# GestaltCogTeam/STEP

Measured on AMD Instinct MI355X. Metric: training windows/sec on PEMS04, horizon-12 MAE parity, 1/2/4/8 MI355X, higher is better.
Workload: dtype f16 (TSFormer Q/K/weights) + bf16 (P, V, GraphWaveNet / graph-learner GEMMs) operands, f32 accumulate

## Files before the change

include/step_hip.h:

```cpp
#ifndef STEP_HIP_H
#define STEP_HIP_H

#include <stdint.h>

#ifdef __cplusplus
extern "C" {
#endif

const char* step_last_error(void);
int step_abi_version(void);

typedef struct StepGemm {
    int M, N, K, batch;
    const void* A; long sam, sak, sab; int a_bf16;
    const void* B; long sbk, sbn, sbb; int b_bf16;
    float* C; long ldc, scn, scb;
    float alpha;
    int accumulate;
    const float* bias; int relu;
    int splitk;
    int a_kblk; long a_kstride;
    int b_kblk; long b_kstride;
    int b_nblk; long b_nstride;
    int c_nblk; long c_nstride;
// ... 13 lines not shown
#define STEP_ENC_WORKGROUPS(n) (((n) & 0xffff) << 8)
int step_tsformer_encode(const float* series, int S, int L, const void* wpack, long wpack_bytes,
                         int depth, int flags, uint16_t* hidden_bf16, float* hidden_f32, float* last_f32,
                         float* sqnorm_part, float dropout_p, const uint64_t* drop_pool, long pool_words, uint64_t seed,
                         unsigned int* fallback_count, void* stream);
int step_dropout_pool_fill(uint64_t* pool, long words, float dropout_p, uint64_t seed, void* stream);
long step_tsformer_dropout_words(int L, int depth);

int step_pack_long_history(const float* x, int B, int L, int N, int C, int ch, float* out, void* stream);
int step_gather_windows(const float* data, int T, int N, int C, int ch, const long* t0, int B, int L, int H,
                        float* long_series, float* hist, float* fut, void* stream);

long step_knn_workspace_bytes(int B, int N, int F);
int step_knn_graph(const uint16_t* hidden, const float* sqnorm_part, int B, int N, int F, int k_total,
                   float* sim, float* adj, void* work, long work_bytes, void* stream);
int step_topk_mask(const float* sim, int B, int N, int k_total, float* adj, void* work, long work_bytes,
                   void* stream);

typedef struct StepDglParams {
    float *conv1_w, *conv1_b;
    float *conv2_w, *conv2_b;
    float *fc_w, *fc_b;
    float *bn1_w, *bn1_b, *bn1_rm, *bn1_rv;
    float *bn2_w, *bn2_b, *bn2_rm, *bn2_rv;
    float *bn3_w, *bn3_b, *bn3_rm, *bn3_rv;
    float *fc_out_w, *fc_out_b;
    float *fc_cat_w, *fc_cat_b;
    int gemm_bf16;
} StepDglParams;

long step_dgl_global_saved_floats(int N, int T);
long step_dgl_global_work_floats(int N, int T, int backward);
int step_dgl_global_forward(const float* series_nt, int N, int T, const StepDglParams* p, int training,
                            float momentum, float* saved, float* work, float* g, void* stream);
int step_dgl_global_backward(const float* series_nt, int N, int T, const StepDglParams* p, const float* saved,
                             const float* dg, float* work, const StepDglParams* grads, void* stream);
#define STEP_DGL_FRESH_FC_GRAD 16
int step_dgl_global_backward_phase(const float* series_nt, int N, int T, const StepDglParams* p, const float* saved,
                             const float* dg, float* work, const StepDglParams* grads, int phase, void* stream);

typedef struct StepDglShard { int own1; double count1, count2; } StepDglShard;
int step_dgl_global_forward_shard(const float* series_slice, int N, int Ts, const StepDglParams* p, int training, float momentum,
                                  float* saved, float* work, double* sums, float* g, const StepDglShard* shard, int phase,
                                  void* stream);
int step_dgl_global_backward_shard(const float* series_slice, int N, int Ts, const StepDglParams* p, const float* saved,
                                   const float* dg, float* work, const StepDglParams* grads, const StepDglShard* shard, int phase,
                                   void* stream);
long step_dgl_global_offset(int N, int T, int item);

long step_dgl_edges_saved_floats(int B, int N);
long step_dgl_edges_work_floats(int N);
long step_dgl_edges_theta_offset(int N);
int step_dgl_edges_forward(const float* g, int N, int B, const StepDglParams* p, const float* u, uint64_t seed,
                           float temperature, float* saved, float* theta_out, float* adj_out, void* stream);
int step_dgl_edges_backward(const float* g, int N, int B, const StepDglParams* p, const float* saved,
                            const float* dtheta, const float* dadj, float temperature, float* work,
                            const StepDglParams* grads, float* dg, void* aux_stream, void* stream);

typedef struct StepGwnetParams {
    float *nodevec1, *nodevec2;
    float *start_w, *start_b;
    float *filter_w[8], *filter_b[8];
    float *gate_w[8], *gate_b[8];
    float *skip_w[8], *skip_b[8];
    float *bn_w[8], *bn_b[8], *bn_rm[8], *bn_rv[8];
    float *gconv_w[8], *gconv_b[8];
    float *fc_his0_w, *fc_his0_b, *fc_his2_w, *fc_his2_b;
    float *end1_w, *end1_b, *end2_w, *end2_b;
    int gemm_bf16;
} StepGwnetParams;

long step_gwnet_saved_floats(int B, int N, int dropout);
long step_gwnet_work_floats(int B, int N, int backward);
long step_gwnet_saved_offset(int B, int N, int dropout, int item, int layer);
int step_gwnet_forward(const float* hist, int B, int N, int Cin, const float* hidden_last, const float* adj,
                       const StepGwnetParams* p, int training, float dropout_p, uint64_t seed, float momentum,
                       float* saved, float* work, float* pred, void* stream);
int step_gwnet_forward_phase(const float* hist, int B, int N, int Cin, const float* hidden_last, const float* adj,
                             const StepGwnetParams* p, int training, float dropout_p, uint64_t seed, float momentum,
                             float* saved, float* work, float* pred, int phase, void* stream);
int step_gwnet_backward(const float* hist, int B, int N, int Cin, const float* hidden_last, const StepGwnetParams* p,
                        const float* saved, float* work, const float* dpred, const StepGwnetParams* grads,
                        float* dadj, int dropout, void* aux_stream, void* leaf_stream, void* stream);

int step_pt_dropout(const float* x, float* y, long n, float p, uint64_t seed, uint32_t site, void* stream);
int step_pt_ffn_hidden_fwd(const float* x, const float* w1, const float* b1, long R, float p, uint64_t seed, uint32_t site,
                           uint16_t* hidden, void* stream);
int step_pt_ffn_hidden_bwd(const float* dy, const float* w2, const uint16_t* hidden, long R, float p, uint16_t* dhidden, void* stream);
int step_pt_colsum_bf16(const uint16_t* x, long rows, int cols, float* out, void* stream);
long step_pt_rows_linear_pack_bytes(int nkc, int nog);
int step_pt_rows_linear_pack(const float* w, long swo, long swi, int nkc, int nog, const float* bias, void* pack, void* stream);
int step_pt_rows_linear(const void* x, int x_bf16, long R, const void* pack, int nkc, int nog, void* y, int y_bf16, int accumulate, void* stream);
int step_pt_layer_pack(const float* wi, const float* bi, const float* wo, const float* bo, const float* w1, const float* b1, const float* w2,
                       const float* b2, void* ffn, void* qkv, void* o, void* da, void* dx, void* stream);
long step_pt_proj_wgrad_ws_floats(long R);
int step_pt_proj_wgrad(const float* x, const uint16_t* dqkv, const float* dov, const uint16_t* a, long R, float* ws, float* dwi, float* dbi, float* dwo,
                       void* stream);
int step_pt_ffn_fused_fwd_ln(const float* h1, long R, const void* pack, float p, const uint64_t* pool, long pool_words, uint64_t seed, uint32_t site_hidden,
                             uint32_t site_out, const float* gamma, const float* beta, float* pre, float* y, float* stats, void* stream);
int step_pt_rows_linear_ln(const uint16_t* x, long R, const void* pack, const float* res, float p, uint64_t seed, uint32_t site, const float* gamma,
                           const float* beta, float* pre, float* y, float* stats, void* stream);
int step_pt_embed_unmasked_fwd(const float* series, const int* um, const float* w, const float* b, const float* pos, long S, int L, int Pu, float p,
                               uint64_t seed, uint32_t site, float* x, void* stream);
int step_pt_embed_unmasked_bwd(const float* dx, const float* series, const int* um, long S, int L, int Pu, float p, uint64_t seed, uint32_t site,
                               float* dpos, float* dw, float* db, void* stream);
int step_pt_dec_input_bwd_sums(const float* dout, long S, int P, int Pu, float p, uint64_t seed, uint32_t site, const int* midx, float* dz, float* dpos,
                               float* dmask, void* stream);
long step_pt_ffn_pack_bytes(void);
long step_pt_ffn_wgrad_workgroups(long R);
long step_pt_ffn_wgrad_ws_floats(long R);
int step_pt_ffn_pack(const float* w1, const float* b1, const float* w2, const float* b2, void* pack, void* stream);
int step_pt_ffn_fused_fwd(const float* h1, long R, const void* pack, float p, const uint64_t* pool, long pool_words, uint64_t seed, uint32_t site,
                          float* f2, void* stream);
int step_pt_ffn_fused_bwd_data(const float* df2, const float* h1, long R, const void* pack, float p, const uint64_t* pool, long pool_words,
                               uint64_t seed, uint32_t site, float* dh1, void* stream);
int step_pt_ffn_fused_bwd_weights(const float* df2, const float* h1, long R, const void* pack, const float* b1, float p, const uint64_t* pool,
                                  long pool_words, uint64_t seed, uint32_t site, float* ws, float* dw1, float* db1, float* dw2, void* stream);
int step_pt_dropout_relu_mask(float* d, const float* relu_of, long n, float p, uint64_t seed, uint32_t site, void* stream);
int step_pt_add_dropout(const float* a, const float* b, float* out, long n, float p, uint64_t seed, uint32_t site, void* stream);
int step_pt_add_rows(float* x, long S, int P, const float* vec, const int* idx, void* stream);
int step_pt_sum_over_seq(const float* dx, long S, int ldp, int p_off, int p_cnt, const int* idx, float* dvec, void* stream);
int step_pt_token_gather(const float* src, long S, int P, const int* idx, int T, float scale, float* dst, void* stream);
int step_pt_token_scatter(const float* ddst, long S, int P, const int* idx, int T, float scale, float* dsrc, void* stream);
int step_pt_dec_input(const float* z, const float* mask_token, const float* pos, const int* midx, long S, int P, int Pu,
                      float p, uint64_t seed, uint32_t site, float* out, void* stream);
int step_pt_dec_input_bwd(const float* dout, long S, int P, int Pu, float p, uint64_t seed, uint32_t site, float* dz,
                          float* dm, void* stream);
int step_pt_layernorm_fwd(const float* x, long R, const float* g, const float* b, float* y, float* stats, void* stream);
int step_pt_layernorm_bwd(const float* dy, const float* x, long R, const float* g, const float* stats, float* dx, float* dgamma,
                          float* dbeta, void* stream);
int step_pt_add_layernorm_fwd(const float* a, const float* b, long R, float p, uint64_t seed, uint32_t site, const float* g,
                              const float* beta, float* pre, float* y, float* stats, void* stream);
int step_pt_layernorm_bwd_dropout(const float* dy, const float* x, long R, const float* g, const float* stats, float* dx,
                                  float* dx_dropped, float p, uint64_t seed, uint32_t site, float* dgamma, float* dbeta,
                                  float* out_colsum, void* stream);
int step_pt_attention_fwd(const float* qkv, long S, int T, float p, uint64_t seed, uint32_t site, float* out, float* stats,
                          void* stream);
int step_pt_attention_bwd(const float* qkv, const float* out, const float* dout, const float* stats, long S, int T, float p,
                          uint64_t seed, uint32_t site, float* dqkv, void* stream);
int step_pt_attention_fwd_bf16(const uint16_t* qkv, long S, int T, float p, uint64_t seed, uint32_t site, uint16_t* out, float* stats,
                               uint32_t* keepbits, const uint64_t* pool, long pool_words, void* stream);
int step_pt_attention_bwd_bf16(const uint16_t* qkv, const uint16_t* out, const uint16_t* dout, const float* stats, long S, int T, float p,
                               uint64_t seed, uint32_t site, uint16_t* dqkv, const uint32_t* keepbits, void* stream);
int step_pt_linear_bf16out(const float* x, const float* w, long swk, long swn, const float* bias, long R, int N, int K, uint16_t* out,
                           void* stream);
int step_pt_relu_mask(float* d, const float* y, long n, void* stream);
int step_colsum(const float* x, long rows, int cols, long ld, float* out, void* stream);

long step_adam_work_floats(void);
int step_adam_clip(float* params, const float* grads, float* exp_avg, float* exp_avg_sq, long n, float lr, float beta1,
                   float beta2, float eps, float weight_decay, int step, float max_norm, float* work, float* out_norm,
                   void* stream);
int step_adam_clip_sharded(float* params, const float* grads, float* exp_avg, float* exp_avg_sq, long n, float lr, float beta1,
                           float beta2, float eps, float weight_decay, int step, float max_norm, const float* extra_sumsq,
                           float* work, float* out_norm, void* stream);
int step_loss_fwd_bwd(const float* pred, const float* real, long n_pred, const float* theta, const float* prior, long n_adj,
                      float null_val, float coef, double* work, float* loss, float* dpred, float* dtheta, void* stream);
int step_loss_scaled_fwd_bwd(const float* pred, const float* real, long n_pred, long real_stride, float scale, float shift,
                             const float* theta, const float* prior, long n_adj, float null_val, float coef, double* work, float* loss,
                             float* dpred, float* dtheta, void* stream);
int step_masked_metrics(const float* pred, long pred_stride, const float* real, long real_stride, long n, float null_val, double* work,
                        float* out, void* stream);
int step_scale2(const float* a, long na, const float* b, long nb, const float* g, float* out_a, float* out_b, void* stream);

typedef struct StepDynState {
    uint64_t seed_xor;
    int32_t adam_step;
    float lr;
    float gsl_coef;
    float reserved;
} StepDynState;
int step_dyn_advance(StepDynState* dyn, void* stream);
int step_dropout_pool_fill_dyn(uint64_t* pool, long words, float dropout_p, uint64_t seed, const StepDynState* dyn, void* stream);
int step_dgl_edges_forward_dyn(const float* g, int N, int B, const StepDglParams* p, const float* u, uint64_t seed,
                               float temperature, float* saved, float* theta_out, float* adj_out, const StepDynState* dyn, void* stream);
int step_gwnet_forward_phase_dyn(const float* hist, int B, int N, int Cin, const float* hidden_last, const float* adj,
                                 const StepGwnetParams* p, int training, float dropout_p, uint64_t seed, float momentum,
                                 float* saved, float* work, float* pred, int phase, const StepDynState* dyn, void* stream);
int step_adam_clip_dyn(float* params, const float* grads, float* exp_avg, float* exp_avg_sq, long n, float beta1, float beta2, float eps,
                       float weight_decay, float max_norm, const float* extra_sumsq, float* work, float* out_norm,
                       const StepDynState* dyn, void* stream);
int step_loss_scaled_fwd_bwd_dyn(const float* pred, const float* real, long n_pred, long real_stride, float scale, float shift,
                                 const float* theta, const float* prior, long n_adj, float null_val, double* work, float* loss,
                                 float* dpred, float* dtheta, const StepDynState* dyn, void* stream);

#define STEP_COMM_ID_BYTES 128
#define STEP_COMM_F32 0
#define STEP_COMM_F64 1
#define STEP_COMM_U8 2
int step_comm_available(void);
int step_comm_version(void);
int step_comm_unique_id(void* id128);
int step_comm_init_rank(const void* id128, int nranks, int rank, void** comm_out);
int step_comm_destroy(void* comm);
int step_comm_set_side_stream(void* comm, void* stream);
int step_comm_allreduce(void* comm, void* buf, long n, int dtype, int average, void* stream);
int step_comm_broadcast(void* comm, void* buf, long n, int dtype, int root, void* stream);
int step_grad_allreduce(void* comm, float* flat_grad, long n, void* stream);
int step_grad_allreduce_begin(void* comm, float* flat_grad, long n, void* stream);
int step_grad_allreduce_join(void* comm, void* stream);

int step_frozen_cache_store(const float* last, const float* adj, int B, int N, const long* slot, long capacity,
                            float* cache_last, uint32_t* cache_bits, void* stream);
int step_frozen_cache_load(const float* cache_last, const uint32_t* cache_bits, long capacity, const long* slot, int B, int N,
                           float* last, float* adj, void* stream);

long step_eval_metrics_acc_doubles(int H);
int step_eval_metrics_accumulate(const float* pred, long p_sb, long p_sh, long p_sn, const float* real, long r_sb, long r_sh, long r_sn,
                                 int B, int H, int N, float scale, float shift, float null_val, double* acc, void* stream);
int step_eval_metrics_finish(const double* acc, int H, double* out, void* stream);

long step_train_tail_work_doubles(void);
int step_train_tail(const float* pred, long p_sb, long p_sh, long p_sn, const float* real, long r_sb, long r_sh, long r_sn, int B, int H,
                    int N, int k, float scale, float shift, float null_val, const float* theta, const float* prior, long n_adj, float coef,
                    double* work, float* loss, float* metrics, float* dpred, float* dtheta, void* stream);

int step_selftest_mfma(int32_t* out, void* stream);
int step_streams_concurrent(void* stream_a, void* stream_b, int* concurrent);

#ifdef __cplusplus
}
#endif
#endif
```

step_amd/_lib.py:

```python
import ctypes
import os

import torch

_HERE = os.path.dirname(os.path.abspath(__file__))
LIB_PATH = os.environ.get("STEP_HIP_LIB") or os.path.join(_HERE, "libstep_hip.so")

_vp, _i, _l, _f, _u64 = ctypes.c_void_p, ctypes.c_int, ctypes.c_long, ctypes.c_float, ctypes.c_uint64


class StepGemm(ctypes.Structure):
    _fields_ = [("M", _i), ("N", _i), ("K", _i), ("batch", _i),
                ("A", _vp), ("sam", _l), ("sak", _l), ("sab", _l), ("a_bf16", _i),
                ("B", _vp), ("sbk", _l), ("sbn", _l), ("sbb", _l), ("b_bf16", _i),
                ("C", _vp), ("ldc", _l), ("scn", _l), ("scb", _l),
                ("alpha", _f), ("accumulate", _i), ("bias", _vp), ("relu", _i), ("splitk", _i),
                ("a_kblk", _i), ("a_kstride", _l), ("b_kblk", _i), ("b_kstride", _l),
                ("b_nblk", _i), ("b_nstride", _l), ("c_nblk", _i), ("c_nstride", _l),
                ("a_kscale", _vp), ("a_kshift", _vp), ("a_kperiod", _i),
                ("batch0", _i), ("sab1", _l), ("sbb1", _l), ("scb1", _l), ("compute_bf16", _i), ("a_rowsum", _vp), ("c_nscale", _vp), ("c_nshift", _vp), ("c_mvec", _vp),
                ("c_nperiod", _i), ("splitk_ws", _vp), ("splitk_ws_floats", _l)]


class StepDglParams(ctypes.Structure):
    NAMES = ["conv1_w", "conv1_b", "conv2_w", "conv2_b", "fc_w", "fc_b",
             "bn1_w", "bn1_b", "bn1_rm", "bn1_rv", "bn2_w", "bn2_b", "bn2_rm", "bn2_rv",
             "bn3_w", "bn3_b", "bn3_rm", "bn3_rv", "fc_out_w", "fc_out_b", "fc_cat_w", "fc_cat_b"]
    _fields_ = [(n, _vp) for n in NAMES] + [("gemm_bf16", _i)]


class StepGwnetParams(ctypes.Structure):
    _fields_ = [("nodevec1", _vp), ("nodevec2", _vp), ("start_w", _vp), ("start_b", _vp),
                ("filter_w", _vp * 8), ("filter_b", _vp * 8), ("gate_w", _vp * 8), ("gate_b", _vp * 8),
                ("skip_w", _vp * 8), ("skip_b", _vp * 8),
                ("bn_w", _vp * 8), ("bn_b", _vp * 8), ("bn_rm", _vp * 8), ("bn_rv", _vp * 8),
                ("gconv_w", _vp * 8), ("gconv_b", _vp * 8),
                ("fc_his0_w", _vp), ("fc_his0_b", _vp), ("fc_his2_w", _vp), ("fc_his2_b", _vp),
                ("end1_w", _vp), ("end1_b", _vp), ("end2_w", _vp), ("end2_b", _vp), ("gemm_bf16", _i)]


_PD = ctypes.POINTER(StepDglParams)


class StepDynState(ctypes.Structure):
    _fields_ = [("seed_xor", ctypes.c_uint64), ("adam_step", ctypes.c_int32), ("lr", _f), ("gsl_coef", _f), ("reserved", _f)]


class StepDglShard(ctypes.Structure):
    _fields_ = [("own1", ctypes.c_int), ("count1", ctypes.c_double), ("count2", ctypes.c_double)]


_PS = ctypes.POINTER(StepDglShard)
_PG = ctypes.POINTER(StepGwnetParams)

_SIGS = {
    "step_last_error": (ctypes.c_char_p, []),
    "step_abi_version": (_i, []),
    "step_gemm": (_i, [ctypes.POINTER(StepGemm), _vp]),
    "step_tsformer_encode": (_i, [_vp, _i, _i, _vp, _l, _i, _i, _vp, _vp, _vp, _vp, _f, _vp, _l, _u64, _vp, _vp]),
    "step_dropout_pool_fill": (_i, [_vp, _l, _f, _u64, _vp]),
    "step_tsformer_dropout_words": (_l, [_i, _i]),
    "step_gather_windows": (_i, [_vp, _i, _i, _i, _i, _vp, _i, _i, _i, _vp, _vp, _vp, _vp]),
    "step_pack_long_history": (_i, [_vp, _i, _i, _i, _i, _i, _vp, _vp]),
    "step_knn_workspace_bytes": (_l, [_i, _i, _i]),
    "step_knn_graph": (_i, [_vp, _vp, _i, _i, _i, _i, _vp, _vp, _vp, _l, _vp]),
    "step_topk_mask": (_i, [_vp, _i, _i, _i, _vp, _vp, _l, _vp]),
    "step_selftest_mfma": (_i, [_vp, _vp]),
    "step_streams_concurrent": (_i, [_vp, _vp, ctypes.POINTER(_i)]),
    "step_dgl_global_saved_floats": (_l, [_i, _i]),
    "step_dgl_global_work_floats": (_l, [_i, _i, _i]),
    "step_dgl_global_forward": (_i, [_vp, _i, _i, _PD, _i, _f, _vp, _vp, _vp, _vp]),
    "step_dgl_global_backward": (_i, [_vp, _i, _i, _PD, _vp, _vp, _vp, _PD, _vp]),
    "step_dgl_global_backward_phase": (_i, [_vp, _i, _i, _PD, _vp, _vp, _vp, _PD, _i, _vp]),
    "step_dgl_global_forward_shard": (_i, [_vp, _i, _i, _PD, _i, _f, _vp, _vp, _vp, _vp, _PS, _i, _vp]),
    "step_dgl_global_backward_shard": (_i, [_vp, _i, _i, _PD, _vp, _vp, _vp, _PD, _PS, _i, _vp]),
    "step_dgl_global_offset": (_l, [_i, _i, _i]),
    "step_dgl_edges_saved_floats": (_l, [_i, _i]),
    "step_dgl_edges_work_floats": (_l, [_i]),
    "step_dgl_edges_theta_offset": (_l, [_i]),
    "step_dgl_edges_forward": (_i, [_vp, _i, _i, _PD, _vp, _u64, _f, _vp, _vp, _vp, _vp]),
    "step_dgl_edges_backward": (_i, [_vp, _i, _i, _PD, _vp, _vp, _vp, _f, _vp, _PD, _vp, _vp, _vp]),
    "step_gwnet_saved_floats": (_l, [_i, _i, _i]),
    "step_gwnet_work_floats": (_l, [_i, _i, _i]),
    "step_gwnet_saved_offset": (_l, [_i, _i, _i, _i, _i]),
    "step_gwnet_forward": (_i, [_vp, _i, _i, _i, _vp, _vp, _PG, _i, _f, _u64, _f, _vp, _vp, _vp, _vp]),
    "step_gwnet_forward_phase": (_i, [_vp, _i, _i, _i, _vp, _vp, _PG, _i, _f, _u64, _f, _vp, _vp, _vp, _i, _vp]),
    "step_gwnet_backward": (_i, [_vp, _i, _i, _i, _vp, _PG, _vp, _vp, _vp, _PG, _vp, _i, _vp, _vp, _vp]),
    "step_pt_dropout": (_i, [_vp, _vp, _l, _f, _u64, ctypes.c_uint32, _vp]),
    "step_pt_ffn_hidden_fwd": (_i, [_vp, _vp, _vp, _l, _f, _u64, ctypes.c_uint32, _vp, _vp]),
    "step_pt_ffn_hidden_bwd": (_i, [_vp, _vp, _vp, _l, _f, _vp, _vp]),
    "step_pt_colsum_bf16": (_i, [_vp, _l, _i, _vp, _vp]),
    "step_pt_rows_linear_pack_bytes": (_l, [_i, _i]),
    "step_pt_rows_linear_pack": (_i, [_vp, _l, _l, _i, _i, _vp, _vp, _vp]),
    "step_pt_rows_linear": (_i, [_vp, _i, _l, _vp, _i, _i, _vp, _i, _i, _vp]),
    "step_pt_layer_pack": (_i, [_vp] * 14),
    "step_pt_proj_wgrad_ws_floats": (_l, [_l]),
    "step_pt_proj_wgrad": (_i, [_vp, _vp, _vp, _vp, _l, _vp, _vp, _vp, _vp, _vp]),
    "step_pt_ffn_fused_fwd_ln": (_i, [_vp, _l, _vp, _f, _vp, _l, _u64, ctypes.c_uint32, ctypes.c_uint32, _vp, _vp, _vp, _vp, _vp, _vp]),
    "step_pt_rows_linear_ln": (_i, [_vp, _l, _vp, _vp, _f, _u64, ctypes.c_uint32, _vp, _vp, _vp, _vp, _vp, _vp]),
    "step_pt_embed_unmasked_fwd": (_i, [_vp, _vp, _vp, _vp, _vp, _l, _i, _i, _f, _u64, ctypes.c_uint32, _vp, _vp]),
    "step_pt_embed_unmasked_bwd": (_i, [_vp, _vp, _vp, _l, _i, _i, _f, _u64, ctypes.c_uint32, _vp, _vp, _vp, _vp]),
    "step_pt_dec_input_bwd_sums": (_i, [_vp, _l, _i, _i, _f, _u64, ctypes.c_uint32, _vp, _vp, _vp, _vp, _vp]),
    "step_pt_ffn_pack_bytes": (_l, []),
    "step_pt_ffn_wgrad_workgroups": (_l, [_l]),
    "step_pt_ffn_wgrad_ws_floats": (_l, [_l]),
    "step_pt_ffn_pack": (_i, [_vp, _vp, _vp, _vp, _vp, _vp]),
    "step_pt_ffn_fused_fwd": (_i, [_vp, _l, _vp, _f, _vp, _l, _u64, ctypes.c_uint32, _vp, _vp]),
    "step_pt_ffn_fused_bwd_data": (_i, [_vp, _vp, _l, _vp, _f, _vp, _l, _u64, ctypes.c_uint32, _vp, _vp]),
    "step_pt_ffn_fused_bwd_weights": (_i, [_vp, _vp, _l, _vp, _vp, _f, _vp, _l, _u64, ctypes.c_uint32, _vp, _vp, _vp, _vp, _vp]),
    "step_pt_add_layernorm_fwd": (_i, [_vp, _vp, _l, _f, _u64, ctypes.c_uint32, _vp, _vp, _vp, _vp, _vp, _vp]),
    "step_pt_layernorm_bwd_dropout": (_i, [_vp, _vp, _l, _vp, _vp, _vp, _vp, _f, _u64, ctypes.c_uint32, _vp, _vp, _vp, _vp]),
    "step_pt_dropout_relu_mask": (_i, [_vp, _vp, _l, _f, _u64, ctypes.c_uint32, _vp]),
    "step_pt_add_dropout": (_i, [_vp, _vp, _vp, _l, _f, _u64, ctypes.c_uint32, _vp]),
    "step_pt_add_rows": (_i, [_vp, _l, _i, _vp, _vp, _vp]),
    "step_pt_sum_over_seq": (_i, [_vp, _l, _i, _i, _i, _vp, _vp, _vp]),
    "step_pt_token_gather": (_i, [_vp, _l, _i, _vp, _i, _f, _vp, _vp]),
    "step_pt_token_scatter": (_i, [_vp, _l, _i, _vp, _i, _f, _vp, _vp]),
    "step_pt_dec_input": (_i, [_vp, _vp, _vp, _vp, _l, _i, _i, _f, _u64, ctypes.c_uint32, _vp, _vp]),
    "step_pt_dec_input_bwd": (_i, [_vp, _l, _i, _i, _f, _u64, ctypes.c_uint32, _vp, _vp, _vp]),
    "step_pt_layernorm_fwd": (_i, [_vp, _l, _vp, _vp, _vp, _vp, _vp]),
    "step_pt_layernorm_bwd": (_i, [_vp, _vp, _l, _vp, _vp, _vp, _vp, _vp, _vp]),
    "step_pt_attention_fwd": (_i, [_vp, _l, _i, _f, _u64, ctypes.c_uint32, _vp, _vp, _vp]),
    "step_pt_attention_bwd": (_i, [_vp, _vp, _vp, _vp, _l, _i, _f, _u64, ctypes.c_uint32, _vp, _vp]),
    "step_pt_attention_fwd_bf16": (_i, [_vp, _l, _i, _f, _u64, ctypes.c_uint32, _vp, _vp, _vp, _vp, _l, _vp]),
    "step_pt_attention_bwd_bf16": (_i, [_vp, _vp, _vp, _vp, _l, _i, _f, _u64, ctypes.c_uint32, _vp, _vp, _vp]),
    "step_pt_linear_bf16out": (_i, [_vp, _vp, _l, _l, _vp, _l, _i, _i, _vp, _vp]),
    "step_pt_relu_mask": (_i, [_vp, _vp, _l, _vp]),
    "step_colsum": (_i, [_vp, _l, _i, _l, _vp, _vp]),
    "step_loss_fwd_bwd": (_i, [_vp, _vp, _l, _vp, _vp, _l, _f, _f, _vp, _vp, _vp, _vp, _vp]),
    "step_loss_scaled_fwd_bwd": (_i, [_vp, _vp, _l, _l, _f, _f, _vp, _vp, _l, _f, _f, _vp, _vp, _vp, _vp, _vp]),
    "step_scale2": (_i, [_vp, _l, _vp, _l, _vp, _vp, _vp, _vp]),
    "step_masked_metrics": (_i, [_vp, _l, _vp, _l, _l, _f, _vp, _vp, _vp]),
    "step_adam_work_floats": (_l, []),
    "step_adam_clip": (_i, [_vp, _vp, _vp, _vp, _l, _f, _f, _f, _f, _f, _i, _f, _vp, _vp, _vp]),
    "step_adam_clip_sharded": (_i, [_vp, _vp, _vp, _vp, _l, _f, _f, _f, _f, _f, _i, _f, _vp, _vp, _vp, _vp]),
    "step_comm_available": (_i, []),
    "step_comm_version": (_i, []),
    "step_comm_unique_id": (_i, [_vp]),
    "step_comm_init_rank": (_i, [_vp, _i, _i, ctypes.POINTER(_vp)]),
    "step_comm_destroy": (_i, [_vp]),
    "step_comm_set_side_stream": (_i, [_vp, _vp]),
    "step_comm_allreduce": (_i, [_vp, _vp, _l, _i, _i, _vp]),
    "step_comm_broadcast": (_i, [_vp, _vp, _l, _i, _i, _vp]),
    "step_grad_allreduce": (_i, [_vp, _vp, _l, _vp]),
    "step_grad_allreduce_begin": (_i, [_vp, _vp, _l, _vp]),
    "step_grad_allreduce_join": (_i, [_vp, _vp]),
    "step_dyn_advance": (_i, [_vp, _vp]),
    "step_dropout_pool_fill_dyn": (_i, [_vp, _l, _f, _u64, _vp, _vp]),
    "step_dgl_edges_forward_dyn": (_i, [_vp, _i, _i, _PD, _vp, _u64, _f, _vp, _vp, _vp, _vp, _vp]),
    "step_gwnet_forward_phase_dyn": (_i, [_vp, _i, _i, _i, _vp, _vp, _PG, _i, _f, _u64, _f, _vp, _vp, _vp, _i, _vp, _vp]),
    "step_adam_clip_dyn": (_i, [_vp, _vp, _vp, _vp, _l, _f, _f, _f, _f, _f, _vp, _vp, _vp, _vp, _vp]),
    "step_loss_scaled_fwd_bwd_dyn": (_i, [_vp, _vp, _l, _l, _f, _f, _vp, _vp, _l, _f, _vp, _vp, _vp, _vp, _vp, _vp]),
    "step_frozen_cache_store": (_i, [_vp, _vp, _i, _i, _vp, _l, _vp, _vp, _vp]),
    "step_frozen_cache_load": (_i, [_vp, _vp, _l, _vp, _i, _i, _vp, _vp, _vp]),
    "step_eval_metrics_acc_doubles": (_l, [_i]),
    "step_eval_metrics_accumulate": (_i, [_vp, _l, _l, _l, _vp, _l, _l, _l, _i, _i, _i, _f, _f, _f, _vp, _vp]),
    "step_eval_metrics_finish": (_i, [_vp, _i, _vp, _vp]),
    "step_train_tail_work_doubles": (_l, []),
    "step_train_tail": (_i, [_vp, _l, _l, _l, _vp, _l, _l, _l, _i, _i, _i, _i, _f, _f, _f, _vp, _vp, _l, _f, _vp, _vp, _vp, _vp, _vp, _vp]),
}

_lib = None


ABI_VERSION = 10
ENC_F16, ENC_ALWAYS_RESHIFT, ENC_RANGE_FLAG = 1, 2, 4
COMM_F32, COMM_F64, COMM_U8, COMM_ID_BYTES = 0, 1, 2, 128


def lib():
    global _lib
    if _lib is None:
        if not os.path.exists(LIB_PATH):
            raise RuntimeError(
                f"libstep_hip.so not found at {LIB_PATH}: build it with `python -m step_amd.build` "
                "(step_amd has no fallback path)")
        _lib = ctypes.CDLL(LIB_PATH)
        for name, (res, args) in _SIGS.items():
            fn = getattr(_lib, name)
            fn.restype = res
            fn.argtypes = args
        if _lib.step_abi_version() != ABI_VERSION:
            v = _lib.step_abi_version()
            _lib = None
            raise RuntimeError(f"libstep_hip.so has ABI version {v}, this package needs {ABI_VERSION}: rebuild with `python -m step_amd.build`")
    return _lib


def exported_symbols():
    return sorted(_SIGS)


def check(rc, what=""):
    if rc != 0:
        msg = lib().step_last_error().decode(errors="replace")
        raise RuntimeError(f"libstep_hip {what} failed (rc={rc}): {msg}")


def ptr(t):
    if t is None:
        return None
    assert t.is_cuda and t.is_contiguous(), "libstep_hip takes contiguous device tensors"
    return ctypes.c_void_p(t.data_ptr())


def stream():
    return ctypes.c_void_p(torch.cuda.current_stream().cuda_stream)


def call(name, *args):
    check(getattr(lib(), name)(*args), name)


# ... 31 lines not shown
```

step_amd/csrc/dgl.hip:

```cpp
#include "common.h"
#include "step_internal.h"

namespace {

constexpr int KW = 10;
constexpr int EMB = 100;

template <int CI, int CO, int TPT>
__global__ __launch_bounds__(256) void conv_relu_fwd_kernel(const float* __restrict__ in, const float* __restrict__ w,
                                                            const float* __restrict__ b, const float* __restrict__ in_sc,
                                                            const float* __restrict__ in_sh, float* __restrict__ out,
                                                            float* __restrict__ partial, int Tin, int stat_limit) {
    __shared__ __attribute__((aligned(16))) float ws[CI * KW * CO];
    __shared__ float red[4][2 * CO];
    const int tid = threadIdx.x, n = blockIdx.y;
    const int Tout = Tin - (KW - 1);
    for (int e = tid; e < CI * KW * CO; e += 256) {
        int co = e % CO, k = (e / CO) % KW, ci = e / (CO * KW);
        ws[e] = w[(co * CI + ci) * KW + k];
    }
    __syncthreads();
    const int t0 = (blockIdx.x * 256 + tid) * TPT;
    float acc[CO][TPT];
#pragma unroll
    for (int co = 0; co < CO; ++co)
#pragma unroll
        for (int j = 0; j < TPT; ++j) acc[co][j] = b[co];
    if (t0 < Tout) {
#pragma unroll 1
        for (int ci = 0; ci < CI; ++ci) {
            const float* src = in + ((long)n * CI + ci) * Tin + t0;
            const float sc = in_sc ? in_sc[ci] : 1.f, sh = in_sh ? in_sh[ci] : 0.f;
            float x[TPT + KW - 1];
#pragma unroll
            for (int q = 0; q < TPT + KW - 1; ++q) x[q] = (t0 + q < Tin) ? src[q] * sc + sh : 0.f;
#pragma unroll
            for (int k = 0; k < KW; ++k) {
                const float* wk = ws + (ci * KW + k) * CO;
#pragma unroll
                for (int co = 0; co < CO; ++co) {
                    const float wv = wk[co];
#pragma unroll
                    for (int j = 0; j < TPT; ++j) acc[co][j] += wv * x[k + j];
                }
            }
        }
    }
    float s1[CO], s2[CO];
#pragma unroll
    for (int co = 0; co < CO; ++co) {
        s1[co] = 0.f; s2[co] = 0.f;
        float* dst = out + ((long)n * CO + co) * Tout + t0;
#pragma unroll
        for (int j = 0; j < TPT; ++j) {
            if (t0 + j < Tout) {
                float v = fmaxf(acc[co][j], 0.f);
                dst[j] = v;
                if (t0 + j < stat_limit) { s1[co] += v; s2[co] += v * v; }
            }
        }
    }
    const int lane = tid & 63, wave = tid >> 6;
#pragma unroll
    for (int co = 0; co < CO; ++co) {
        float a = wave_sum(s1[co]), q = wave_sum(s2[co]);
        if (lane == 0) { red[wave][co] = a; red[wave][CO + co] = q; }
    }
    __syncthreads();
    if (tid < 2 * CO)
        partial[((long)blockIdx.y * gridDim.x + blockIdx.x) * (2 * CO) + tid] = red[0][tid] + red[1][tid] + red[2][tid] + red[3][tid];
}

__global__ __launch_bounds__(256) void bn_finalize_kernel(const float* __restrict__ partial, int nblk, int C, double count,
                                                          const float* __restrict__ gamma, const float* __restrict__ beta,
                                                          float* __restrict__ rmean, float* __restrict__ rvar, int training,
                                                          float momentum, float* __restrict__ stat) {
    __shared__ double r1[256], r2[256];
    const int c = blockIdx.x, tid = threadIdx.x;
    double mean, var;
    if (training) {
        double a = 0.0, q = 0.0;
        for (int i = tid; i < nblk; i += 256) { a += partial[(long)i * 2 * C + c]; q += partial[(long)i * 2 * C + C + c]; }
        r1[tid] = a; r2[tid] = q;
        __syncthreads();
        for (int s = 128; s > 0; s >>= 1) {
            if (tid < s) { r1[tid] += r1[tid + s]; r2[tid] += r2[tid + s]; }
            __syncthreads();
        }
        mean = r1[0] / count;
        var = fmax(r2[0] / count - mean * mean, 0.0);
        if (tid == 0) {
            rmean[c] = (1.f - momentum) * rmean[c] + momentum * (float)mean;
            rvar[c] = (1.f - momentum) * rvar[c] + momentum * (float)(var * count / fmax(count - 1.0, 1.0));
        }
    } else {
        mean = rmean[c];
        var = rvar[c];
    }
    if (tid == 0) {
        float rstd = (float)(1.0 / sqrt(var + 1e-5));
        float sc = gamma[c] * rstd;
        stat[c] = sc;
        stat[C + c] = beta[c] - (float)mean * sc;
        stat[2 * C + c] = (float)mean;
        stat[3 * C + c] = rstd;
    }
}

__global__ __launch_bounds__(256) void bn_sums_kernel(const float* __restrict__ partial, int nblk, int C, double* __restrict__ sums) {
    __shared__ double r1[256], r2[256];
    const int c = blockIdx.x, tid = threadIdx.x;
    double a = 0.0, q = 0.0;
    for (int i = tid; i < nblk; i += 256) { a += partial[(long)i * 2 * C + c]; q += partial[(long)i * 2 * C + C + c]; }
    r1[tid] = a; r2[tid] = q;
    __syncthreads();
    for (int s = 128; s > 0; s >>= 1) {
        if (tid < s) { r1[tid] += r1[tid + s]; r2[tid] += r2[tid + s]; }
        __syncthreads();
    }
    if (tid == 0) { sums[c] = r1[0]; sums[C + c] = r2[0]; }
}
__global__ __launch_bounds__(256) void bn_sums_sliced_kernel(const float* __restrict__ partial, int nblk, int C, double* __restrict__ sums) {
    __shared__ double r1[256], r2[256];
    const int c = blockIdx.x, tid = threadIdx.x;
    const int per = (nblk + gridDim.y - 1) / gridDim.y, beg = blockIdx.y * per, end = min(nblk, beg + per);
    double a = 0.0, q = 0.0;
    for (int i = beg + tid; i < end; i += 256) { a += partial[(long)i * 2 * C + c]; q += partial[(long)i * 2 * C + C + c]; }
    r1[tid] = a; r2[tid] = q;
    __syncthreads();
    for (int s = 128; s > 0; s >>= 1) {
        if (tid < s) { r1[tid] += r1[tid + s]; r2[tid] += r2[tid + s]; }
        __syncthreads();
    }
    if (tid == 0) { unsafeAtomicAdd(sums + c, r1[0]); unsafeAtomicAdd(sums + C + c, r2[0]); }
}
__global__ void bn_finalize_sums_kernel(const double* __restrict__ sums, int C, double count, const float* __restrict__ gamma,
                                        const float* __restrict__ beta, float* __restrict__ rmean, float* __restrict__ rvar,
                                        int training, float momentum, float* __restrict__ stat) {
    const int c = threadIdx.x;
    if (c >= C) return;
    double mean, var;
    if (training) {
        mean = sums[c] / count;
        var = fmax(sums[C + c] / count - mean * mean, 0.0);
        rmean[c] = (1.f - momentum) * rmean[c] + momentum * (float)mean;
        rvar[c] = (1.f - momentum) * rvar[c] + momentum * (float)(var * count / fmax(count - 1.0, 1.0));
    } else {
        mean = rmean[c]; var = rvar[c];
    }
    const float rstd = (float)(1.0 / sqrt(var + 1e-5));
    const float sc = gamma[c] * rstd;
    stat[c] = sc; stat[C + c] = beta[c] - (float)mean * sc; stat[2 * C + c] = (float)mean; stat[3 * C + c] = rstd;
}

__global__ __launch_bounds__(256) void fc_post_bn3_kernel(float* __restrict__ gpre, const float* __restrict__ bias, int N,
                                                          const float* __restrict__ gamma, const float* __restrict__ beta,
                                                          float* __restrict__ rmean, float* __restrict__ rvar, int training,
                                                          float momentum, float* __restrict__ stat, float* __restrict__ g) {
    __shared__ double r1[256], r2[256];
    const int j = blockIdx.x, tid = threadIdx.x;
    const float bj = bias[j];
    double a = 0.0, q = 0.0;
    for (int n = tid; n < N; n += 256) {
        float v = gpre[(long)n * EMB + j] + bj;
        gpre[(long)n * EMB + j] = v;
        v = fmaxf(v, 0.f);
        a += v; q += (double)v * v;
    }
    r1[tid] = a; r2[tid] = q;
    __syncthreads();
    for (int s = 128; s > 0; s >>= 1) {
        if (tid < s) { r1[tid] += r1[tid + s]; r2[tid] += r2[tid + s]; }
        __syncthreads();
    }
    double mean, var;
    if (training) {
        mean = r1[0] / N;
        var = fmax(r2[0] / N - mean * mean, 0.0);
        if (tid == 0) {
            rmean[j] = (1.f - momentum) * rmean[j] + momentum * (float)mean;
            rvar[j] = (1.f - momentum) * rvar[j] + momentum * (float)(var * N / fmax((double)N - 1.0, 1.0));
        }
    } else {
        mean = rmean[j]; var = rvar[j];
    }
    const float rstd = (float)(1.0 / sqrt(var + 1e-5));
    if (tid == 0) { stat[2 * EMB + j] = (float)mean; stat[3 * EMB + j] = rstd; }
    const float sc = gamma[j] * rstd, sh = beta[j] - (float)mean * sc;
    for (int n = tid; n < N; n += 256) g[(long)n * EMB + j] = fmaxf(gpre[(long)n * EMB + j], 0.f) * sc + sh;
}

__global__ __launch_bounds__(256) void bn3_relu_bwd_kernel(const float* __restrict__ dg, const float* __restrict__ gpre, int N,
                                                           const float* __restrict__ gamma, const float* __restrict__ stat,
                                                           float* __restrict__ dgamma, float* __restrict__ dbeta,
                                                           float* __restrict__ dbias, float* __restrict__ dgpre,
                                                           float* __restrict__ dgpreT, float* __restrict__ colsum) {
    __shared__ double r1[256], r2[256];
    const int j = blockIdx.x, tid = threadIdx.x;
    const float mean = stat[2 * EMB + j], rstd = stat[3 * EMB + j];
    double a = 0.0, q = 0.0;
    for (int n = tid; n < N; n += 256) {
        float d = dg[(long)n * EMB + j];
        float xh = (fmaxf(gpre[(long)n * EMB + j], 0.f) - mean) * rstd;
        a += d; q += (double)d * xh;
    }
    r1[tid] = a; r2[tid] = q;
    __syncthreads();
    for (int s = 128; s > 0; s >>= 1) {
        if (tid < s) { r1[tid] += r1[tid + s]; r2[tid] += r2[tid + s]; }
        __syncthreads();
    }
    const float m1 = (float)(r1[0] / N), m2 = (float)(r2[0] / N);
    const float k = gamma[j] * rstd;
    __syncthreads();
    double sb = 0.0;
    for (int n = tid; n < N; n += 256) {
        float pre = gpre[(long)n * EMB + j];
        float xh = (fmaxf(pre, 0.f) - mean) * rstd;
        float dh = k * (dg[(long)n * EMB + j] - m1 - xh * m2);
        float v = pre > 0.f ? dh : 0.f;
        dgpre[(long)n * EMB + j] = v;
        dgpreT[(long)j * N + n] = v;
        sb += v;
    }
    if (tid == 0) { dgamma[j] += (float)r2[0]; dbeta[j] += (float)r1[0]; }
    __syncthreads();
    r1[tid] = sb;
    __syncthreads();
    for (int s = 128; s > 0; s >>= 1) {
        if (tid < s) r1[tid] += r1[tid + s];
        __syncthreads();
    }
    if (tid == 0) { dbias[j] += (float)r1[0]; colsum[j] = (float)r1[0]; }
}

template <int C>
__global__ __launch_bounds__(256) void bn_bwd_reduce_kernel(const float* __restrict__ dy, const float* __restrict__ x,
                                                            const float* __restrict__ stat, int Tlen, float* __restrict__ partial) {
    __shared__ float red[4][2];
    const int n = blockIdx.z, c = blockIdx.y, tid = threadIdx.x;
    const float mean = stat[2 * C + c], rstd = stat[3 * C + c];
    const long base = ((long)n * C + c) * Tlen;
    float a = 0.f, q = 0.f;
    for (int t = blockIdx.x * 1024 + tid; t < min(Tlen, (int)(blockIdx.x + 1) * 1024); t += 256) {
        float d = dy[base + t];
        a += d; q += d * ((x[base + t] - mean) * rstd);
    }
    a = wave_sum(a); q = wave_sum(q);
    if ((tid & 63) == 0) { red[tid >> 6][0] = a; red[tid >> 6][1] = q; }
    __syncthreads();
    if (tid < 2) {
        long blk = (long)n * gridDim.x + blockIdx.x;
        partial[(blk * C + c) * 2 + tid] = red[0][tid] + red[1][tid] + red[2][tid] + red[3][tid];
    }
}
__global__ __launch_bounds__(256) void bn_bwd_finalize_kernel(const float* __restrict__ partial, int nblk, int C, double count,
                                                              const float* __restrict__ gamma, const float* __restrict__ stat,
                                                              float* __restrict__ dgamma, float* __restrict__ dbeta,
                                                              float* __restrict__ coef) {
    __shared__ double r1[256], r2[256];
    const int c = blockIdx.x, tid = threadIdx.x;
    double a = 0.0, q = 0.0;
    for (int i = tid; i < nblk; i += 256) { a += partial[((long)i * C + c) * 2]; q += partial[((long)i * C + c) * 2 + 1]; }
    r1[tid] = a; r2[tid] = q;
    __syncthreads();
    for (int s = 128; s > 0; s >>= 1) {
        if (tid < s) { r1[tid] += r1[tid + s]; r2[tid] += r2[tid + s]; }
        __syncthreads();
    }
    if (tid == 0) {
        dgamma[c] += (float)r2[0];
        dbeta[c] += (float)r1[0];
        coef[c] = (float)(r1[0] / count);
        coef[C + c] = (float)(r2[0] / count);
        coef[2 * C + c] = gamma[c] * stat[3 * C + c];
    }
}
template <int C>
__global__ __launch_bounds__(256) void bn_bwd_apply_kernel(float* __restrict__ dy, const float* __restrict__ x,
                                                           const float* __restrict__ stat, const float* __restrict__ coef, int Tlen) {
    const int n = blockIdx.z, c = blockIdx.y;
// ... 358 lines not shown
__global__ void gpre_init_kernel(float* __restrict__ gpre, const float* __restrict__ shiftdot, long n) {
    const long i = (long)blockIdx.x * 256 + threadIdx.x;
    if (i < n) gpre[i] = shiftdot[i % EMB];
}
__global__ __launch_bounds__(256) void fc_unpermute_kernel(const float* __restrict__ graw, const float* __restrict__ fc_w,
                                                           const float* __restrict__ st2, const float* __restrict__ colsum,
                                                           float* __restrict__ dfc_w, float* __restrict__ dots_o, int T2, int overwrite) {
    __shared__ float red[4][32];
    const int o = blockIdx.y, t = blockIdx.x * 256 + threadIdx.x, tid = threadIdx.x;
    const float cso = colsum[o];
    float d[32];
#pragma unroll
    for (int i = 0; i < 32; ++i) d[i] = 0.f;
    if (t < T2) {
        const float4* src = (const float4*)(graw + ((long)o * T2 + t) * 16);
        const float4 g0 = src[0], g1 = src[1], g2 = src[2], g3 = src[3];
        const float g[16] = {g0.x, g0.y, g0.z, g0.w, g1.x, g1.y, g1.z, g1.w, g2.x, g2.y, g2.z, g2.w, g3.x, g3.y, g3.z, g3.w};
        float w[16], old[16];
#pragma unroll
        for (int c = 0; c < 16; ++c) { const long idx = ((long)o * 16 + c) * T2 + t; w[c] = fc_w[idx]; old[c] = overwrite ? 0.f : dfc_w[idx]; }
#pragma unroll
        for (int c = 0; c < 16; ++c) {
            dfc_w[((long)o * 16 + c) * T2 + t] = old[c] + st2[c] * g[c] + st2[16 + c] * cso;
            d[2 * c] = w[c] * g[c]; d[2 * c + 1] = w[c] * cso;
        }
    }
#pragma unroll
    for (int i = 0; i < 32; ++i) {
        const float v = wave_sum(d[i]);
        if ((tid & 63) == 0) red[tid >> 6][i] = v;
    }
    __syncthreads();
    if (tid < 32) atomicAdd(&dots_o[o * 32 + tid], red[0][tid] + red[1][tid] + red[2][tid] + red[3][tid]);
}
__global__ void dots_reduce_kernel(const float* __restrict__ dots_o, float* __restrict__ dots) {
    const int i = threadIdx.x;
    if (i >= 32) return;
    double a = 0.0;
    for (int o = 0; o < EMB; ++o) a += dots_o[o * 32 + i];
    dots[i] = (float)a;
}

static bool dgl_channels_last(const StepDglParams* p) {
    const char* e = getenv("STEP_DGL_F32_STORAGE");
    return p->gemm_bf16 && !(e && e[0] == '1');
}

static bool dgl_legacy_bn_backward() {
    const char* e = getenv("STEP_DGL_LEGACY_BN");
    return e && e[0] == '1';
}

extern "C" long step_dgl_global_saved_floats(int N, int T) {
    long T1 = T - 9, T2 = T - 18;
    return (long)N * 8 * T1 + (long)N * 16 * T2 + (long)N * EMB + 4 * 8 + 4 * 16 + 4 * EMB + (long)EMB * 16 * T2 + 128;
}
static long fc_splitk_ws_floats(int N, int T2) {
    const int splits = step_gemm_auto_splitk(N, EMB, 16 * T2, 1);
    return splits > 1 ? (long)splits * N * EMB + 4 : 0;
}
extern "C" long step_dgl_global_work_floats(int N, int T, int backward) {
    long T1 = T - 9, T2 = T - 18;
    long nb1 = (long)N * cdiv(T1, 1024), nb2 = (long)N * cdiv(T2, 1024);
    long part = (nb1 > nb2 ? nb1 : nb2) * 32 + 64;
    if (!backward) return part + dgl_conv2_pack_floats() + 64 + fc_splitk_ws_floats(N, (int)T2);
    return part + (long)N * 16 * T2 + (long)N * 8 * T1 + (long)EMB * 16 * T2 + 2L * N * EMB + DGL_SMALL + dgl_conv2_wgrad_scratch_floats(N, (int)T1);
}

static float* saved_wp(float* saved, int N, int T) {
    long T1 = T - 9, T2 = T - 18;
    return saved + (long)N * 8 * T1 + (long)N * 16 * T2 + (long)N * EMB + 4 * 8 + 4 * 16 + 4 * EMB;
}
static void carve_saved(float* saved, int N, int T, float** a1, float** a2, float** gpre, float** st1, float** st2, float** st3) {
    long T1 = T - 9, T2 = T - 18;
    *a1 = saved; saved += (long)N * 8 * T1;
    *a2 = saved; saved += (long)N * 16 * T2;
    *gpre = saved; saved += (long)N * EMB;
    *st1 = saved; saved += 4 * 8;
    *st2 = saved; saved += 4 * 16;
    *st3 = saved;
}

static int dgl_bn_stats(const float* partial, int nblk, int C, double count, const float* gamma, const float* beta, float* rm, float* rv,
                        int training, float momentum, float* stat, double* sums, hipStream_t st) {
    if (nblk < 8192) {
        bn_finalize_kernel<<<C, 256, 0, st>>>(partial, nblk, C, count, gamma, beta, rm, rv, training, momentum, stat);
    } else {
        if (hipMemsetAsync(sums, 0, 2 * C * sizeof(double), st) != hipSuccess) { step_set_error("memset failed"); return STEP_ERR_HIP; }
        bn_sums_sliced_kernel<<<dim3(C, 32), 256, 0, st>>>(partial, nblk, C, sums);
        bn_finalize_sums_kernel<<<1, 64, 0, st>>>(sums, C, count, gamma, beta, rm, rv, training, momentum, stat);
    }
    STEP_LAUNCH_CHECK("bn_stats");
    return STEP_OK;
}

static int dgl_global_forward_impl(const float* series_nt, int N, int T, const StepDglParams* p, int training, float momentum,
                                   float* saved, float* work, double* sums, float* g, const StepDglShard* shard, int phase,
                                   hipStream_t st) {
    const int T1 = T - 9, T2 = T - 18;
    float *a1, *a2, *gpre, *st1, *st2, *st3;
    carve_saved(saved, N, T, &a1, &a2, &gpre, &st1, &st2, &st3);
    float* partial = work;
    const bool all = phase == 0;
    const double count1 = shard ? shard->count1 : (double)N * T1, count2 = shard ? shard->count2 : (double)N * T2;
    const bool cl = dgl_channels_last(p);
    const long part_floats = ((long)N * cdiv(T1, 1024) > (long)N * cdiv(T2, 1024) ? (long)N * cdiv(T1, 1024) : (long)N * cdiv(T2, 1024)) * 32 + 64;
    double* own_sums = (double*)(work + part_floats + dgl_conv2_pack_floats());
    float* wp = saved_wp(saved, N, T);
    float* shiftdot = wp + (long)EMB * 16 * T2;
    if (all || phase == 1) {
        int nblk;
        if (cl) {
            STEP_TRY(dgl_conv1_fwd_cl(series_nt, p->conv1_w, p->conv1_b, a1, partial, N, T, shard ? shard->own1 : T1, &nblk, st));
        } else {
            dim3 grid(cdiv(T1, 256 * 4), N);
            conv_relu_fwd_kernel<1, 8, 4><<<grid, 256, 0, st>>>(series_nt, p->conv1_w, p->conv1_b, nullptr, nullptr, a1, partial, T,
                                                                shard ? shard->own1 : T1);
            STEP_LAUNCH_CHECK("conv1");
            nblk = grid.x * grid.y;
        }
        if (shard) bn_sums_kernel<<<8, 256, 0, st>>>(partial, nblk, 8, sums);
        else STEP_TRY(dgl_bn_stats(partial, nblk, 8, count1, p->bn1_w, p->bn1_b, p->bn1_rm, p->bn1_rv, training, momentum, st1, own_sums, st));
        STEP_LAUNCH_CHECK("bn1");
    }
    if (all || phase == 2) {
        if (shard) bn_finalize_sums_kernel<<<1, 64, 0, st>>>(sums, 8, count1, p->bn1_w, p->bn1_b, p->bn1_rm, p->bn1_rv, training, momentum, st1);
        int nblk;
        if (cl) {
            STEP_TRY(dgl_conv2_fwd_cl(a1, p->conv2_w, p->conv2_b, st1, st1 + 8, a2, partial, N, T1, &nblk,
                                      work + part_floats, st));
        } else if (p->gemm_bf16) {
            STEP_TRY(dgl_conv2_fwd_mfma(a1, p->conv2_w, p->conv2_b, st1, st1 + 8, a2, partial, N, T1, &nblk, st));
        } else {
            dim3 grid(cdiv(T2, 256 * 4), N);
            conv_relu_fwd_kernel<8, 16, 4><<<grid, 256, 0, st>>>(a1, p->conv2_w, p->conv2_b, st1, st1 + 8, a2, partial, T1, T2);
            STEP_LAUNCH_CHECK("conv2");
            nblk = grid.x * grid.y;
        }
        if (shard) bn_sums_kernel<<<16, 256, 0, st>>>(partial, nblk, 16, sums + 16);
        else STEP_TRY(dgl_bn_stats(partial, nblk, 16, count2, p->bn2_w, p->bn2_b, p->bn2_rm, p->bn2_rv, training, momentum, st2, own_sums, st));
        STEP_LAUNCH_CHECK("bn2");
    }
    if (all || phase == 3) {
        if (shard) bn_finalize_sums_kernel<<<1, 64, 0, st>>>(sums + 16, 16, count2, p->bn2_w, p->bn2_b, p->bn2_rm, p->bn2_rv, training, momentum, st2);
        const long K = 16L * T2;
        StepGemm gm = gemm_desc(N, EMB, (int)K, a2, K, 1, p->fc_w, 1, K, gpre, EMB);
        if (cl) {
            if (hipMemsetAsync(shiftdot, 0, 128 * sizeof(float), st) != hipSuccess) { step_set_error("memset failed"); return STEP_ERR_HIP; }
            fc_prep_kernel<<<dim3(cdiv(T2, 256), EMB), 256, 0, st>>>(p->fc_w, st2, (uint4*)wp, shiftdot, T2);
            gpre_init_kernel<<<cdiv((long)N * EMB, 256), 256, 0, st>>>(gpre, shiftdot, (long)N * EMB);
            STEP_LAUNCH_CHECK("fc_prep");
            gm.a_bf16 = 1;
            gm.B = wp; gm.b_bf16 = 1;
        } else {
            if (hipMemsetAsync(gpre, 0, (size_t)N * EMB * sizeof(float), st) != hipSuccess) { step_set_error("memset failed"); return STEP_ERR_HIP; }
            gm.a_kscale = st2; gm.a_kshift = st2 + 16; gm.a_kperiod = T2;
        }
        gm.accumulate = 2;
        gm.splitk = -1;
        gm.compute_bf16 = p->gemm_bf16;
        if (fc_splitk_ws_floats(N, T2) > 0) {
            float* ws = work + part_floats + dgl_conv2_pack_floats() + 64;
            gm.splitk_ws = (float*)(((uintptr_t)ws + 15) & ~(uintptr_t)15);
            gm.splitk_ws_floats = fc_splitk_ws_floats(N, T2) - 4;
        }
        STEP_TRY(step_gemm_launch(gm, st));
    }
    if (all || phase == 4) {
        fc_post_bn3_kernel<<<EMB, 256, 0, st>>>(gpre, p->fc_b, N, p->bn3_w, p->bn3_b, p->bn3_rm, p->bn3_rv, training, momentum, st3, g);
        STEP_LAUNCH_CHECK("fc_post_bn3");
    }
    return STEP_OK;
}

extern "C" int step_dgl_global_forward(const float* series_nt, int N, int T, const StepDglParams* p, int training,
                                       float momentum, float* saved, float* work, float* g, void* stream) {
    STEP_REQUIRE(series_nt && p && saved && work && g && N > 0 && T > 18, "dgl_global_forward: bad arguments");
    return dgl_global_forward_impl(series_nt, N, T, p, training, momentum, saved, work, nullptr, g, nullptr, 0, (hipStream_t)stream);
}

extern "C" int step_dgl_global_forward_shard(const float* series_slice, int N, int Ts, const StepDglParams* p, int training,
                                             float momentum, float* saved, float* work, double* sums, float* g,
                                             const StepDglShard* shard, int phase, void* stream) {
    STEP_REQUIRE(series_slice && p && saved && work && sums && g && shard && N > 0 && Ts > 18 && phase >= 1 && phase <= 4,
                 "dgl_global_forward_shard: bad arguments");
    STEP_REQUIRE(shard->own1 > 0 && shard->own1 <= Ts - 9 && shard->count1 > 0 && shard->count2 > 0, "dgl_global_forward_shard: bad shard");
    return dgl_global_forward_impl(series_slice, N, Ts, p, training, momentum, saved, work, sums, g, shard, phase, (hipStream_t)stream);
}

extern "C" long step_dgl_global_offset(int N, int T, int item) {
    const long T1 = T - 9, T2 = T - 18;
    if (item == 0) return 0;
    if (item == 1) return (long)N * 8 * T1;
    if (item == 2) return (long)N * 8 * T1 + (long)N * 16 * T2;
    const long nb1 = (long)N * cdiv(T1, 1024), nb2 = (long)N * cdiv(T2, 1024);
    const long coef = (nb1 > nb2 ? nb1 : nb2) * 32 + 64 + (long)N * 16 * T2 + (long)N * 8 * T1 + (long)EMB * 16 * T2 + 2L * N * EMB;
    if (item == 10) return coef + 256;
    if (item == 11) return coef + 320;
    return -1;
}

static int dgl_global_backward_impl(const float* series_nt, int N, int T, const StepDglParams* p, const float* saved, const float* dg,
                                    float* work, const StepDglParams* grads, const StepDglShard* shard, int phase, void* stream);

extern "C" int step_dgl_global_backward(const float* series_nt, int N, int T, const StepDglParams* p, const float* saved,
                                        const float* dg, float* work, const StepDglParams* grads, void* stream) {
    return step_dgl_global_backward_phase(series_nt, N, T, p, saved, dg, work, grads, 0, stream);
}

extern "C" int step_dgl_global_backward_phase(const float* series_nt, int N, int T, const StepDglParams* p, const float* saved,
                                              const float* dg, float* work, const StepDglParams* grads, int phase, void* stream) {
    STEP_REQUIRE(series_nt && p && saved && dg && work && grads && N > 0 && T > 18 && (phase & ~STEP_DGL_FRESH_FC_GRAD) >= 0 &&
                 (phase & ~STEP_DGL_FRESH_FC_GRAD) <= 2, "dgl_global_backward: bad arguments");
    return dgl_global_backward_impl(series_nt, N, T, p, saved, dg, work, grads, nullptr, phase, stream);
}

extern "C" int step_dgl_global_backward_shard(const float* series_slice, int N, int Ts, const StepDglParams* p, const float* saved,
                                              const float* dg, float* work, const StepDglParams* grads, const StepDglShard* shard,
                                              int phase, void* stream) {
    const int ph = phase & ~STEP_DGL_FRESH_FC_GRAD;
    STEP_REQUIRE(series_slice && p && saved && dg && work && grads && shard && N > 0 && Ts > 18 && (ph == 1 || ph == 3 || ph == 4),
                 "dgl_global_backward_shard: bad arguments");
    STEP_REQUIRE(p->gemm_bf16 && Ts - 18 >= 128, "dgl_global_backward_shard: needs the bf16 contraction mode and a slice of >= 128 conv2 columns");
    return dgl_global_backward_impl(series_slice, N, Ts, p, saved, dg, work, grads, shard, phase, stream);
}

static int dgl_global_backward_impl(const float* series_nt, int N, int T, const StepDglParams* p, const float* saved, const float* dg,
                                    float* work, const StepDglParams* grads, const StepDglShard* shard, int phase, void* stream) {
    const int fresh_fc = (phase & STEP_DGL_FRESH_FC_GRAD) ? 1 : 0;
    phase &= ~STEP_DGL_FRESH_FC_GRAD;
    const bool do_fc = phase == 0 || phase == 1, do_mid = phase == 0 || phase == 2 || phase == 3, do_tail = phase == 0 || phase == 2 || phase == 4;
    hipStream_t st = (hipStream_t)stream;
    const int T1 = T - 9, T2 = T - 18;
    const long K = 16L * T2;
    float *a1, *a2, *gpre, *st1, *st2, *st3;
    carve_saved((float*)saved, N, T, &a1, &a2, &gpre, &st1, &st2, &st3);
    long nb1 = (long)N * cdiv(T1, 1024), nb2 = (long)N * cdiv(T2, 1024);
    float* partial = work;
    float* d_a2 = work + (nb1 > nb2 ? nb1 : nb2) * 32 + 64;
    float* d_a1 = d_a2 + (long)N * 16 * T2;
    float* wraw = d_a1 + (long)N * 8 * T1;
    float* dgpre = wraw + (long)EMB * K;
    float* dgpreT = dgpre + (long)N * EMB;
    float* coef = dgpreT + (long)N * EMB;
    float* dots = coef + 256;
    float* graw = coef + 320;
    float* wg_scratch = coef + DGL_SMALL;
    const bool fuse2 = T2 >= 128 && (shard || !dgl_legacy_bn_backward());
    const double count1 = shard ? shard->count1 : (double)N * T1, count2 = shard ? shard->count2 : (double)N * T2;
    if (dgl_channels_last(p)) {
        const float* wp = saved_wp((float*)saved, N, T);
        float* dots_o = coef + 256 + 64 + 1344;
        float* colsum = coef + 128;
        if (do_fc) {
            bn3_relu_bwd_kernel<<<EMB, 256, 0, st>>>(dg, gpre, N, p->bn3_w, st3, grads->bn3_w, grads->bn3_b, grads->fc_b, dgpre, dgpreT, colsum);
            STEP_LAUNCH_CHECK("bn3_bwd");
            StepGemm gm = gemm_desc(EMB, (int)K, N, dgpre, 1, EMB, a2, K, 1, wraw, K);
            gm.b_bf16 = 1;
            gm.compute_bf16 = 1;
            STEP_TRY(step_gemm_launch(gm, st));
            if (hipMemsetAsync(dots_o, 0, EMB * 32 * sizeof(float), st) != hipSuccess) { step_set_error("memset failed"); return STEP_ERR_HIP; }
            fc_unpermute_kernel<<<dim3(cdiv(T2, 256), EMB), 256, 0, st>>>(wraw, p->fc_w, st2, colsum, grads->fc_w, dots_o, T2, fresh_fc);
            dots_reduce_kernel<<<1, 64, 0, st>>>(dots_o, dots);
            STEP_LAUNCH_CHECK("fc_unpermute");
        }
        if (do_mid) {
            bn2_fused_coef_kernel<<<1, 64, 0, st>>>(dots, st2, p->bn2_w, count2, grads->bn2_w, grads->bn2_b, coef);
            STEP_LAUNCH_CHECK("bn2_fused_coef");
            StepGemm gm = gemm_desc(N, (int)K, EMB, dgpre, EMB, 1, wp, K, 1, d_a2, K);
            gm.b_bf16 = 1;
            gm.compute_bf16 = 1;
            GemmFused fu = {nullptr, nullptr, a2, coef, st2, 16, T2, GEMM_FUSED_INTERLEAVED};
            STEP_TRY(step_gemm_launch_fused(gm, fu, st));
            STEP_TRY(dgl_conv2_wgrad_cl(d_a2, a1, wg_scratch, graw, N, T1, st));
        }
        if (do_tail) {
            STEP_TRY(dgl_conv2_wgrad_finish(graw, p->conv2_w, st1, p->bn1_w, p->bn1_b, count1, grads->conv2_w, grads->conv2_b, grads->bn1_w,
                                            grads->bn1_b, coef + 64, 1, st));
            STEP_TRY(dgl_conv2_dgrad_cl(d_a2, p->conv2_w, st1, d_a1, N, T1, a1, coef + 64, st1, shard ? shard->own1 : T1, wraw, st));
            STEP_TRY(dgl_conv1_wgrad_cl(d_a1, series_nt, wg_scratch, grads->conv1_w, grads->conv1_b, N, T, st));
        }
        return STEP_OK;
    }
    if (do_fc) {
        float* colsum = coef + 128;
        bn3_relu_bwd_kernel<<<EMB, 256, 0, st>>>(dg, gpre, N, p->bn3_w, st3, grads->bn3_w, grads->bn3_b, grads->fc_b, dgpre, dgpreT, colsum);
        STEP_LAUNCH_CHECK("bn3_bwd");
        {
            StepGemm gm = gemm_desc(EMB, (int)K, N, dgpre, 1, EMB, a2, K, 1, grads->fc_w, K);
            gm.accumulate = fresh_fc ? 0 : 1;
            gm.c_nscale = st2; gm.c_nshift = st2 + 16; gm.c_nperiod = T2; gm.c_mvec = colsum;
            gm.compute_bf16 = p->gemm_bf16;
            if (fuse2) {
                if (hipMemsetAsync(dots, 0, 32 * sizeof(float), st) != hipSuccess) { step_set_error("memset failed"); return STEP_ERR_HIP; }
                GemmFused fu = {p->fc_w, dots, nullptr, nullptr, nullptr, 16, T2};
                STEP_TRY(step_gemm_launch_fused(gm, fu, st));
            } else {
                STEP_TRY(step_gemm_launch(gm, st));
            }
        }
    }
    if (!do_mid && !do_tail) return STEP_OK;
    if (do_mid) {
        StepGemm gm = gemm_desc(N, (int)K, EMB, dgpreT, 1, N, p->fc_w, K, 1, d_a2, K);
        if (p->gemm_bf16 || fuse2) { gm.A = dgpre; gm.sam = EMB; gm.sak = 1; }
        gm.compute_bf16 = p->gemm_bf16;
        if (fuse2) {
            bn2_fused_coef_kernel<<<1, 64, 0, st>>>(dots, st2, p->bn2_w, count2, grads->bn2_w, grads->bn2_b, coef);
            STEP_LAUNCH_CHECK("bn2_fused_coef");
            GemmFused fu = {nullptr, nullptr, a2, coef, st2, 16, T2};
            STEP_TRY(step_gemm_launch_fused(gm, fu, st));
        } else {
            STEP_TRY(step_gemm_launch(gm, st));
        }
    }
    if (do_mid && !fuse2) {
        dim3 grid(cdiv(T2, 1024), 16, N);
        bn_bwd_reduce_kernel<16><<<grid, 256, 0, st>>>(d_a2, a2, st2, T2, partial);
        STEP_LAUNCH_CHECK("bn2_bwd_reduce");
        bn_bwd_finalize_kernel<<<16, 256, 0, st>>>(partial, (int)nb2, 16, (double)N * T2, p->bn2_w, st2, grads->bn2_w, grads->bn2_b, coef);
        STEP_LAUNCH_CHECK("bn2_bwd_finalize");
        bn_bwd_apply_kernel<16><<<grid, 256, 0, st>>>(d_a2, a2, st2, coef, T2);
        STEP_LAUNCH_CHECK("bn2_bwd_apply");
    }
    const bool fuse1 = p->gemm_bf16 && (shard || !dgl_legacy_bn_backward());
    if (fuse1) {
        if (do_mid) STEP_TRY(dgl_conv2_wgrad_xhat_mfma(d_a2, a1, st1, wg_scratch, graw, N, T1, st));
        if (!do_tail) return STEP_OK;
        STEP_TRY(dgl_conv2_wgrad_finish(graw, p->conv2_w, st1, p->bn1_w, p->bn1_b, count1, grads->conv2_w, grads->conv2_b, grads->bn1_w,
                                        grads->bn1_b, coef + 64, 0, st));
        STEP_TRY(dgl_conv2_dgrad_mfma(d_a2, p->conv2_w, d_a1, N, T1, a1, coef + 64, st1, shard ? shard->own1 : T1, st));
    } else if (p->gemm_bf16) {
        STEP_TRY(dgl_conv2_wgrad_mfma(d_a2, a1, st1, st1 + 8, wg_scratch, grads->conv2_w, grads->conv2_b, N, T1, st));
        STEP_TRY(dgl_conv2_dgrad_mfma(d_a2, p->conv2_w, d_a1, N, T1, nullptr, nullptr, nullptr, T1, st));
    } else {
        conv_bwd_weight_kernel<8, 16><<<N, 256, 0, st>>>(d_a2, a1, st1, st1 + 8, grads->conv2_w, grads->conv2_b, T1);
        STEP_LAUNCH_CHECK("conv2_bwd_weight");
        conv_bwd_data_kernel<8, 16, 4><<<dim3(cdiv(T1, 1024), N), 256, 0, st>>>(d_a2, p->conv2_w, d_a1, T1);
        STEP_LAUNCH_CHECK("conv2_bwd_data");
    }
    if (!fuse1) {
        dim3 grid(cdiv(T1, 1024), 8, N);
        bn_bwd_reduce_kernel<8><<<grid, 256, 0, st>>>(d_a1, a1, st1, T1, partial);
        STEP_LAUNCH_CHECK("bn1_bwd_reduce");
// ... 98 lines not shown
```

step_amd/csrc/gwnet.hip:

```cpp
#include "common.h"
#include "step_internal.h"
#include <vector>

namespace {

constexpr int C = 32, CAT = 224, CS = 256, CE = 512, OUT = 12, NL = 8, HID = 96;
constexpr int TIN[NL] = {13, 12, 10, 9, 7, 6, 4, 3};
constexpr int DIL[NL] = {1, 2, 1, 2, 1, 2, 1, 2};
constexpr int TOUT[NL] = {12, 10, 9, 7, 6, 4, 3, 1};

__global__ void start_conv_kernel(const float* __restrict__ hist, int B, int N, int Cin, const float* __restrict__ w,
                                  const float* __restrict__ b, float* __restrict__ x0) {
    long idx = (long)blockIdx.x * 256 + threadIdx.x;
    long total = (long)B * N * 13 * C;
    if (idx >= total) return;
    int c = idx % C, t = (idx / C) % 13;
    long bn = idx / (C * 13);
    int n = bn % N, bb = bn / N;
    float v = b[c];
    if (t >= 1) {
        const float* src = hist + (((long)bb * 12 + (t - 1)) * N + n) * Cin;
        v += w[c * 2] * src[0] + w[c * 2 + 1] * src[1];
    }
    x0[idx] = v;
}
__global__ __launch_bounds__(256) void start_conv_bwd_kernel(const float* __restrict__ hist, int B, int N, int Cin,
                                                             const float* __restrict__ dx0, float* __restrict__ dw,
                                                             float* __restrict__ db) {
    __shared__ float red[8][96];
    const int c = threadIdx.x & 31;
    const int sub = threadIdx.x >> 5;
    long npos = (long)B * N * 13;
    float a0 = 0.f, a1 = 0.f, ab = 0.f;
    for (long p = (long)blockIdx.x * 8 + sub; p < npos; p += (long)gridDim.x * 8) {
        int t = p % 13;
        long bn = p / 13;
        int n = bn % N, bb = bn / N;
        float d = dx0[p * C + c];
        ab += d;
        if (t >= 1) {
            const float* src = hist + (((long)bb * 12 + (t - 1)) * N + n) * Cin;
            a0 += d * src[0]; a1 += d * src[1];
        }
    }
    red[sub][c] = a0; red[sub][32 + c] = a1; red[sub][64 + c] = ab;
    __syncthreads();
    if (threadIdx.x < 96) {
        float s = 0.f;
#pragma unroll
        for (int r = 0; r < 8; ++r) s += red[r][threadIdx.x];
        const int cc = threadIdx.x & 31, kind = threadIdx.x >> 5;
        if (kind == 2) atomicAdd(&db[cc], s); else atomicAdd(&dw[cc * 2 + kind], s);
    }
}

__global__ __launch_bounds__(256) void row_sums_kernel(const float* __restrict__ A, int N, float* __restrict__ rs, float* __restrict__ cs_init) {
    __shared__ float red[4];
    const long row = blockIdx.x;
    float s = 0.f;
    for (int j = threadIdx.x; j < N; j += 256) s += A[row * N + j];
    s = wave_sum(s);
    if ((threadIdx.x & 63) == 0) red[threadIdx.x >> 6] = s;
    __syncthreads();
    if (threadIdx.x == 0) { rs[row] = 1.f + red[0] + red[1] + red[2] + red[3]; cs_init[row] = 1.f; }
}
__global__ __launch_bounds__(256) void col_sums_kernel(const float* __restrict__ A, int N, float* __restrict__ cs) {
    __shared__ float red[4][64];
    const int b = blockIdx.z;
    const int j = blockIdx.x * 64 + (threadIdx.x & 63), w = threadIdx.x >> 6;
    const int per = (N + gridDim.y - 1) / gridDim.y, ibeg = blockIdx.y * per, iend = min(N, ibeg + per);
    float s = 0.f;
    if (j < N)
        for (int i = ibeg + w; i < iend; i += 4) s += A[((long)b * N + i) * N + j];
    red[w][threadIdx.x & 63] = s;
    __syncthreads();
    if (w == 0 && j < N) atomicAdd(&cs[(long)b * N + j], red[0][threadIdx.x] + red[1][threadIdx.x] + red[2][threadIdx.x] + red[3][threadIdx.x]);
}
__global__ __launch_bounds__(256) void rw_build_kernel(const float* __restrict__ A, int N, const float* __restrict__ rs,
                                                       const float* __restrict__ cs, float* __restrict__ Pf, float* __restrict__ Pb,
                                                       float* __restrict__ PfT, float* __restrict__ PbT) {
    __shared__ float tile[32][33];
    const int b = blockIdx.z, i0 = blockIdx.y * 32, j0 = blockIdx.x * 32;
    const int tx = threadIdx.x & 31, ty = threadIdx.x >> 5;
    const long base = (long)b * N * N;
    for (int r = ty; r < 32; r += 8) {
        int i = i0 + r, j = j0 + tx;
        float a = (i < N && j < N) ? A[base + (long)i * N + j] : 0.f;
        tile[r][tx] = a;
        if (i < N && j < N) {
            const float v = a + (i == j ? 1.f : 0.f);
            Pf[base + (long)i * N + j] = v / rs[(long)b * N + i];
            PbT[base + (long)i * N + j] = v / cs[(long)b * N + j];
        }
    }
    __syncthreads();
    for (int r = ty; r < 32; r += 8) {
        int j = j0 + r, i = i0 + tx;
        if (i < N && j < N) {
            const float v = tile[tx][r] + (i == j ? 1.f : 0.f);
            Pb[base + (long)j * N + i] = v / cs[(long)b * N + j];
            PfT[base + (long)j * N + i] = v / rs[(long)b * N + i];
        }
    }
}
__global__ void replicate_adp_kernel(const float* __restrict__ Pa, int N, int B, float* __restrict__ P2, float* __restrict__ PT2) {
    long idx = (long)blockIdx.x * 256 + threadIdx.x;
    if (idx >= (long)N * N) return;
    int i = idx / N, j = idx % N;
    float v = Pa[idx], vt = Pa[(long)j * N + i];
    for (int b = 0; b < B; ++b) { P2[(long)b * N * N + idx] = v; PT2[(long)b * N * N + idx] = vt; }
}
__global__ void stacks_to_bf16_kernel(const float* __restrict__ P, const float* __restrict__ PT, long rows, int N, int N8,
                                      uint16_t* __restrict__ P16, uint16_t* __restrict__ PT16) {
    long idx = (long)blockIdx.x * 256 + threadIdx.x;
    if (idx >= rows * (N8 / 2)) return;
    const long row = idx / (N8 / 2);
    const int j = (int)(idx % (N8 / 2)) * 2;
    const float* src = blockIdx.y ? PT : P;
    uint16_t* dst = blockIdx.y ? PT16 : P16;
    const float a = j < N ? src[row * N + j] : 0.f, b = j + 1 < N ? src[row * N + j + 1] : 0.f;
    typedef __attribute__((ext_vector_type(2))) float f2;
    typedef __attribute__((ext_vector_type(2))) __bf16 b2;
    f2 t = {a, b};
    *(uint32_t*)(dst + row * N8 + j) = __builtin_bit_cast(uint32_t, __builtin_convertvector(t, b2));
}
__global__ __launch_bounds__(256) void slots_to_bf16T_kernel(const float* __restrict__ cat, int slot0, int sstep, int B, int N, int T, int N8,
                                                             uint16_t* __restrict__ XT) {
    __shared__ float tile[64][33];
    const int v0 = blockIdx.x * 64, t = blockIdx.y, src = blockIdx.z / B, b = blockIdx.z % B;
    const int slot = slot0 + sstep * src;
    const int c = threadIdx.x & 31, r = threadIdx.x >> 5;
    for (int i = r; i < 64; i += 8) {
        const int v = v0 + i;
        tile[i][c] = v < N ? cat[(((long)b * N + v) * T + t) * CAT + slot * C + c] : 0.f;
    }
    __syncthreads();
    const int cc = threadIdx.x >> 3, g8 = (threadIdx.x & 7) * 8;
    if (v0 + g8 < N8) {
        float v8[8];
#pragma unroll
        for (int j = 0; j < 8; ++j) v8[j] = tile[g8 + j][cc];
        *(bf16x8*)(XT + (((long)blockIdx.z * T + t) * C + cc) * N8 + v0 + g8) = pack8(v8);
    }
}
__global__ void sum_batches_kernel(const float* __restrict__ x, long n, int B, float* __restrict__ out) {
    long idx = (long)blockIdx.x * 256 + threadIdx.x;
    if (idx >= n) return;
    float s = 0.f;
    for (int b = 0; b < B; ++b) s += x[(long)b * n + idx];
    out[idx] = s;
}
__global__ __launch_bounds__(256) void row_dot_kernel(const float* __restrict__ dP, const float* __restrict__ P, int N,
                                                      float* __restrict__ out) {
    __shared__ float red[4];
    const long row = blockIdx.x;
    float s = 0.f;
    for (int j = threadIdx.x; j < N; j += 256) s += dP[row * N + j] * P[row * N + j];
    s = wave_sum(s);
    if ((threadIdx.x & 63) == 0) red[threadIdx.x >> 6] = s;
    __syncthreads();
    if (threadIdx.x == 0) out[row] = red[0] + red[1] + red[2] + red[3];
}
__global__ __launch_bounds__(256) void rw_bwd_kernel(const float* __restrict__ dPf, const float* __restrict__ dPb, int N,
                                                     const float* __restrict__ rs, const float* __restrict__ cs,
                                                     const float* __restrict__ rf, const float* __restrict__ rb, float* __restrict__ dA) {
    __shared__ float tile[32][33];
    const int b = blockIdx.z, i0 = blockIdx.y * 32, j0 = blockIdx.x * 32;
    const int tx = threadIdx.x & 31, ty = threadIdx.x >> 5;
    const long base = (long)b * N * N;
    for (int r = ty; r < 32; r += 8) {
        int j = j0 + r, i = i0 + tx;
        tile[r][tx] = (i < N && j < N) ? (dPb[base + (long)j * N + i] - rb[(long)b * N + j]) / cs[(long)b * N + j] : 0.f;
    }
    __syncthreads();
    for (int r = ty; r < 32; r += 8) {
        int i = i0 + r, j = j0 + tx;
        if (i < N && j < N)
            dA[base + (long)i * N + j] = (dPf[base + (long)i * N + j] - rf[(long)b * N + i]) / rs[(long)b * N + i] + tile[tx][r];
    }
}
__global__ __launch_bounds__(256) void softmax_relu_rows_kernel(const float* __restrict__ M, int N, float* __restrict__ P) {
    __shared__ float red[4];
    const long row = blockIdx.x;
    float mx = 0.f;
    for (int j = threadIdx.x; j < N; j += 256) mx = fmaxf(mx, M[row * N + j]);
    mx = wave_max(mx);
    if ((threadIdx.x & 63) == 0) red[threadIdx.x >> 6] = mx;
    __syncthreads();
    mx = fmaxf(fmaxf(red[0], red[1]), fmaxf(red[2], red[3]));
    __syncthreads();
    float s = 0.f;
    for (int j = threadIdx.x; j < N; j += 256) s += __expf(fmaxf(M[row * N + j], 0.f) - mx);
    s = wave_sum(s);
    if ((threadIdx.x & 63) == 0) red[threadIdx.x >> 6] = s;
    __syncthreads();
    const float inv = 1.f / (red[0] + red[1] + red[2] + red[3]);
    for (int j = threadIdx.x; j < N; j += 256) P[row * N + j] = __expf(fmaxf(M[row * N + j], 0.f) - mx) * inv;
}
__global__ void softmax_relu_bwd_kernel(const float* __restrict__ M, const float* __restrict__ P, const float* __restrict__ dP,
                                        const float* __restrict__ rdot, int N, float* __restrict__ dM) {
    long idx = (long)blockIdx.x * 256 + threadIdx.x;
    if (idx >= (long)N * N) return;
    int i = idx / N;
    dM[idx] = M[idx] > 0.f ? P[idx] * (dP[idx] - rdot[i]) : 0.f;
}

struct GatePtrs { float *wf[8], *bf[8], *wg[8], *bg[8]; };
struct SkipPtrs { float *w[8], *b[8]; };
struct MixPtrs { const float* w[7]; };
__global__ __launch_bounds__(256) void pack_weights_kernel(GatePtrs P, SkipPtrs K, MixPtrs M, float* __restrict__ wcat_all,
                                                           float* __restrict__ wcatT_all, float* __restrict__ bcat_all,
                                                           float* __restrict__ wskip, float* __restrict__ bsum, float* __restrict__ wmixT) {
    const int blk = blockIdx.x, tid = threadIdx.x;
    if (blk < 128) {
        const int L = blk >> 4;
        const int idx = (blk & 15) * 256 + tid;
        const int o = idx / 64, k = idx % 64;
        const float v = (o < 32 ? P.wf[L] : P.wg[L])[(((o & 31) * 32) + (k & 31)) * 2 + (k >> 5)];
        wcat_all[L * 4096 + idx] = v;
        wcatT_all[L * 4096 + k * 64 + o] = v;
        if (idx < 64) bcat_all[L * 64 + idx] = idx < 32 ? P.bf[L][idx] : P.bg[L][idx - 32];
    } else if (blk < 384) {
        const int o = blk - 128, k = tid;
        wskip[o * CS + k] = K.w[k >> 5][o * C + (k & 31)];
        if (o == 0) {
            float sum = 0.f;
#pragma unroll
            for (int i = 0; i < 8; ++i) sum += K.b[i][k];
            bsum[k] = sum;
        }
    } else {
        const int L = (blk - 384) / 28;
        const int idx = ((blk - 384) % 28) * 256 + tid;
        const int c = idx / CAT, j = idx % CAT;
        wmixT[L * (C * CAT) + j * C + c] = M.w[L][idx];
    }
}
__global__ void unpack_gate_grad_kernel(const float* __restrict__ dwcat_all, const float* __restrict__ dbcat_all, GatePtrs G) {
    const int L = blockIdx.y;
    const float* dwcat = dwcat_all + L * 4096;
    const float* dbcat = dbcat_all + L * 64;
    float *dwf = G.wf[L], *dbf = G.bf[L], *dwg = G.wg[L], *dbg = G.bg[L];
    int idx = blockIdx.x * 256 + threadIdx.x;
    if (idx < 64 * 64) {
// ... 604 lines not shown
        if (i > 0) {
            bn.gamma = p->bn_w[i - 1]; bn.beta = p->bn_b[i - 1]; bn.rm = p->bn_rm[i - 1]; bn.rv = p->bn_rv[i - 1];
            bn.stat = S.bnstat[i - 1]; bn.sums = W.acc64 + (long)(i - 1) * NCOPY * 64;
        }
        if (!(i == 0 && skip_first_tcn)) {
            tcn_fwd_kernel<BF16><<<(unsigned)cdiv(npos, 128), 256, 0, st>>>(i == 0 ? S.x0 : S.y[i - 1], bn, npos, Tin, Tout, dil, W.wcat + i * 4096,
                                                                            W.bcat + i * 64, S.tf[i], S.sg[i], S.cat[i], S.zlast, i);
            STEP_LAUNCH_CHECK("tcn_fwd");
        }
        if (first_tcn_only) break;
        if (i == NL - 1 && !(dead_bn7 && training)) break;
        STEP_TRY(nconv_fwd3(S.Pstk, S.PT16, S.cat[i], 0, 0, 1, B, N, Tout, BF16, W.xT, st));
        STEP_TRY(nconv_fwd3(S.Pstk, S.PT16, S.cat[i], 1, 2, 2, B, N, Tout, BF16, W.xT, st));
        const XIn xin = {i == 0 ? S.x0 : S.y[i - 1], i == 0 ? nullptr : S.bnstat[i - 1]};
        const bool dead = i == NL - 1;
        mix_fwd_kernel<BF16><<<(unsigned)cdiv(npos, 64), 256, 0, st>>>(S.cat[i], p->gconv_w[i], p->gconv_b[i], xin, npos, Tin, Tout, dil, drop_p,
                                                                       (uint32_t)seed, (uint32_t)(seed >> 32), (uint32_t)i, dead ? W.m7 : S.mask[i],
                                                                       dead ? W.y7 : S.y[i], W.acc64 + (long)i * NCOPY * 64, dyn);
        STEP_LAUNCH_CHECK("mix_fwd");
        if (dead) {
            const BnFwd b7 = {p->bn_w[i], p->bn_b[i], p->bn_rm[i], p->bn_rv[i], 1, momentum, S.bnstat[i], (double)npos, W.acc64 + (long)i * NCOPY * 64};
            bn_stats_only_kernel<<<1, 64, 0, st>>>(b7);
            STEP_LAUNCH_CHECK("bn7_stats");
        }
    }
    return STEP_OK;
}

static int pack_weights(const StepGwnetParams* p, const Work& W, hipStream_t st) {
    GatePtrs gp;
    SkipPtrs sp;
    MixPtrs mp;
    for (int i = 0; i < NL; ++i) {
        gp.wf[i] = p->filter_w[i]; gp.bf[i] = p->filter_b[i]; gp.wg[i] = p->gate_w[i]; gp.bg[i] = p->gate_b[i];
        sp.w[i] = p->skip_w[i]; sp.b[i] = p->skip_b[i];
        if (i < NL - 1) mp.w[i] = p->gconv_w[i];
    }
    pack_weights_kernel<<<384 + 7 * 28, 256, 0, st>>>(gp, sp, mp, W.wcat, W.wcatT, W.bcat, W.wskip, W.bsum, W.wmixT);
    STEP_LAUNCH_CHECK("pack_weights");
    return STEP_OK;
}

extern "C" int step_gwnet_forward(const float* hist, int B, int N, int Cin, const float* hidden_last, const float* adj,
                                  const StepGwnetParams* p, int training, float dropout_p, uint64_t seed, float momentum,
                                  float* saved, float* work, float* pred, void* stream) {
    return step_gwnet_forward_phase(hist, B, N, Cin, hidden_last, adj, p, training, dropout_p, seed, momentum, saved, work, pred, 0, stream);
}

extern "C" int step_gwnet_forward_phase(const float* hist, int B, int N, int Cin, const float* hidden_last, const float* adj,
                                        const StepGwnetParams* p, int training, float dropout_p, uint64_t seed, float momentum,
                                        float* saved, float* work, float* pred, int phase, void* stream) {
    return step_gwnet_forward_phase_dyn(hist, B, N, Cin, hidden_last, adj, p, training, dropout_p, seed, momentum, saved, work, pred, phase, nullptr,
                                        stream);
}
extern "C" int step_gwnet_forward_phase_dyn(const float* hist, int B, int N, int Cin, const float* hidden_last, const float* adj,
                                            const StepGwnetParams* p, int training, float dropout_p, uint64_t seed, float momentum,
                                            float* saved, float* work, float* pred, int phase, const StepDynState* dyn, void* stream) {
    STEP_REQUIRE(p && saved && work && phase >= 0 && phase <= 6, "gwnet_forward: null argument / bad phase");
    const bool do_prep = phase == 0 || phase == 1 || phase == 5, do_layers = phase == 0 || phase == 1 || phase == 6;
    const bool do_his = phase == 0 || phase == 2 || phase == 3, do_head = phase == 0 || phase == 2 || phase == 4;
    STEP_REQUIRE(!do_prep || hist, "gwnet_forward: the layer phase needs hist");
    STEP_REQUIRE(!do_layers || adj, "gwnet_forward: the layer phase needs adj");
    STEP_REQUIRE(!do_his || hidden_last, "gwnet_forward: the fc_his phase needs hidden_last");
    STEP_REQUIRE(!do_head || pred, "gwnet_forward: the head phase needs pred");
    STEP_REQUIRE(B > 0 && N > 0 && Cin >= 2, "gwnet_forward: bad sizes B=%d N=%d C=%d", B, N, Cin);
    hipStream_t st = (hipStream_t)stream;
    const bool train = (training & 1) != 0;
    const bool use_drop = train && dropout_p > 0.f;
    Saved S = carve_saved(saved, B, N, use_drop);
    Work W = carve_work(work, B, N, false);
    const long BN = (long)B * N;
    const int allbf16 = p->gemm_bf16;

    const long NN = (long)N * N;
    const bool dead_bn7 = (training & 2) != 0;
    if (do_prep) {
        STEP_TRY(zero((float*)W.acc64, 2L * NL * NCOPY * 64, st));
        start_conv_kernel<<<g1(BN * 13 * C), 256, 0, st>>>(hist, B, N, Cin, p->start_w, p->start_b, S.x0);
        STEP_LAUNCH_CHECK("start_conv");
        {
            StepGemm g = gemm_desc(N, N, 10, p->nodevec1, 10, 1, p->nodevec2, N, 1, S.Madp, N);
            STEP_TRY(step_gemm_launch(g, st));
            softmax_relu_rows_kernel<<<N, 256, 0, st>>>(S.Madp, N, S.Pa);
            replicate_adp_kernel<<<g1(NN), 256, 0, st>>>(S.Pa, N, B, S.Pstk + 2 * B * NN, S.PTstk + 2 * B * NN);
            STEP_LAUNCH_CHECK("adp_softmax");
        }
        STEP_TRY(pack_weights(p, W, st));
        if (allbf16) STEP_TRY(gwnet_layers_forward<true>(p, S, W, B, N, train, use_drop ? dropout_p : 0.f, seed, momentum, dead_bn7, dyn, st, true, false));
        else STEP_TRY(gwnet_layers_forward<false>(p, S, W, B, N, train, use_drop ? dropout_p : 0.f, seed, momentum, dead_bn7, dyn, st, true, false));
    }
    if (do_layers) {
        row_sums_kernel<<<(unsigned)BN, 256, 0, st>>>(adj, N, S.rs, S.cs);
        {
            int slices = cdiv(512, cdiv(N, 64) * B);
            if (slices > cdiv(N, 64)) slices = cdiv(N, 64);
            if (slices < 1) slices = 1;
            col_sums_kernel<<<dim3(cdiv(N, 64), slices, B), 256, 0, st>>>(adj, N, S.cs);
        }
        rw_build_kernel<<<dim3(cdiv(N, 32), cdiv(N, 32), B), 256, 0, st>>>(adj, N, S.rs, S.cs, S.Pstk, S.Pstk + B * NN, S.PTstk,
                                                                           S.PTstk + B * NN);
        STEP_LAUNCH_CHECK("rw_build");
        if (p->gemm_bf16) {
            const long rows = 3L * B * N;
            stacks_to_bf16_kernel<<<dim3((unsigned)cdiv(rows * (n8(N) / 2), 256), 2), 256, 0, st>>>(S.Pstk, S.PTstk, rows, N, n8(N), S.P16,
                                                                                                   S.PT16);
            STEP_LAUNCH_CHECK("stacks_to_bf16");
        }
        if (allbf16) STEP_TRY(gwnet_layers_forward<true>(p, S, W, B, N, train, use_drop ? dropout_p : 0.f, seed, momentum, dead_bn7, dyn, st, false, true));
        else STEP_TRY(gwnet_layers_forward<false>(p, S, W, B, N, train, use_drop ? dropout_p : 0.f, seed, momentum, dead_bn7, dyn, st, false, true));
    }

    if (do_his) {
        StepGemm g = gemm_desc((int)BN, CE, HID, hidden_last, HID, 1, p->fc_his0_w, 1, HID, S.h1, CE);
        g.bias = p->fc_his0_b; g.relu = 1;
        g.compute_bf16 = allbf16; STEP_TRY(step_gemm_launch(g, st));
        StepGemm g2 = gemm_desc((int)BN, CS, CE, S.h1, CE, 1, p->fc_his2_w, 1, CE, S.h2, CS);
        g2.bias = p->fc_his2_b; g2.relu = 1;
        g2.compute_bf16 = allbf16; STEP_TRY(step_gemm_launch(g2, st));
    }
    if (do_head) {
        StepGemm gs = gemm_desc((int)BN, CS, CS, S.zlast, CS, 1, W.wskip, 1, CS, S.skip, CS);
        gs.bias = W.bsum;
        gs.compute_bf16 = allbf16; STEP_TRY(step_gemm_launch(gs, st));
        head_combine_kernel<<<g1(BN * CS), 256, 0, st>>>(S.skip, S.h2, BN * CS, S.xh);
        STEP_LAUNCH_CHECK("head_combine");
        StepGemm g3 = gemm_desc((int)BN, CE, CS, S.xh, CS, 1, p->end1_w, 1, CS, S.e1, CE);
        g3.bias = p->end1_b; g3.relu = 1;
        g3.compute_bf16 = allbf16; STEP_TRY(step_gemm_launch(g3, st));
        StepGemm g4 = gemm_desc(N, OUT, CE, S.e1, CE, 1, p->end2_w, 1, CE, pred, 1);
        g4.batch = B; g4.sab = (long)N * CE; g4.scb = (long)OUT * N; g4.scn = N;
        g4.bias = p->end2_b;
        g4.compute_bf16 = allbf16; STEP_TRY(step_gemm_launch(g4, st));
    }
    return STEP_OK;
}

template <bool BF16>
static int gwnet_layers_backward(const StepGwnetParams* p, const StepGwnetParams* grads, const Saved& S, const Work& W, int B, int N,
                                 float** dx0, hipStream_t st, AuxLane& lane, AuxLane& leaves, hipEvent_t* adj_done) {
    const long BN = (long)B * N;
    float* dx_next = nullptr;
    float* dxbuf[2] = {W.dxa, W.dxb};
    {
        AdjOffsets o;
        for (int i = 0; i < NL - 1; ++i) { o.cat[i] = S.cat[i] - S.cat[0]; o.dcat[i] = W.dcat[i] - W.dcat[0]; }
        adj_ktab_kernel<<<3, 128, 0, st>>>(o, N, W.ktab);
        STEP_LAUNCH_CHECK("adj_ktab");
    }
    static const bool adj_pieces = []() { const char* e = getenv("STEP_ADJ_PIECES"); return !(e && e[0] == '0'); }();
    bool adj_first = true;
    auto adj_piece = [&](int lo, int hi, hipStream_t on_stream) -> int {
        int seg0 = 0, nseg = 0;
        for (int i = 0; i < lo; ++i) seg0 += 2 * TOUT[i];
        for (int i = lo; i <= hi; ++i) nseg += 2 * TOUT[i];
        StepGemm g = gemm_desc(N, N, 32 * nseg, S.cat[0], 0, 1, W.dcat[0], 1, 0, W.dPstk, N);
        g.batch = 3 * B; g.batch0 = B;
        g.scb = (long)N * N; g.scb1 = (long)B * N * N;
        g.compute_bf16 = BF16;
        g.accumulate = adj_first ? 0 : 1;
        adj_first = false;
        return step_gemm_segmented_launch(g, W.ktab + seg0, ADJ_NSEG, on_stream);
    };
    for (int i = NL - 1; i >= 0; --i) {
        const int Tin = TIN[i], Tout = TOUT[i], dil = DIL[i];
        const long npos = BN * Tout;
        const float* cat = S.cat[i];
        if (i < NL - 1) {
            const BnBwd bn = {p->bn_w[i], S.bnstat[i], grads->bn_w[i], grads->bn_b[i], (double)npos, W.acc64 + (long)i * NCOPY * 64};
            mix_bwd_kernel<BF16><<<(unsigned)cdiv(npos, 128), 256, 0, st>>>(dx_next, S.y[i], bn, S.mask[i], W.wmixT + i * (C * CAT), npos, W.dres, W.dh[i],
                                                                            W.dcat[i]);
            STEP_LAUNCH_CHECK("mix_bwd");
            STEP_TRY(nconv_bwd_data3(S.PTstk, S.P16, W.dcat[i], 2, 1, 2, B, N, Tout, BF16, W.xT, st));
            STEP_TRY(nconv_bwd_data3(S.PTstk, S.P16, W.dcat[i], 1, 0, 0, B, N, Tout, BF16, W.xT, st));
            if (adj_pieces && i == 0) { STEP_TRY(adj_piece(0, 0, lane.fork())); *adj_done = lane.done(); }
        }
        float* dx = dxbuf[i & 1];
        tcn_bwd_kernel<BF16><<<(unsigned)cdiv(BN, TB_ROWS / Tout), 256, 0, st>>>(i < NL - 1 ? W.dcat[i] : nullptr, W.dskip, i, S.tf[i], S.sg[i],
                                                                                W.wcatT + i * 4096, i < NL - 1 ? W.dres : nullptr, BN, Tin, Tout, dil,
                                                                                W.dpre[i], dx, i > 0 ? S.y[i - 1] : nullptr,
                                                                                i > 0 ? S.bnstat[i - 1] : nullptr,
                                                                                i > 0 ? W.acc64 + (long)(i - 1) * NCOPY * 64 : nullptr);
        STEP_LAUNCH_CHECK("tcn_bwd");
        const XIn xin = {i == 0 ? S.x0 : S.y[i - 1], i == 0 ? nullptr : S.bnstat[i - 1]};
        hipEvent_t ev = leaves.on ? leaves.mark() : lane.mark();
        if (adj_pieces && i == 4) STEP_TRY(adj_piece(4, 6, lane.after(ev)));
        if (adj_pieces && i == 2) STEP_TRY(adj_piece(2, 3, lane.after(ev)));
        if (adj_pieces && i == 1) STEP_TRY(adj_piece(1, 1, lane.after(ev)));
        hipStream_t leaf = leaves.after(ev);
        if (i < NL - 1) {
            StepGemm gw = gemm_desc(C, CAT, (int)npos, W.dh[i], 1, C, cat, CAT, 1, grads->gconv_w[i], CAT);
            gw.accumulate = 2; gw.splitk = -1;
            gw.a_rowsum = grads->gconv_b[i];
            gw.compute_bf16 = BF16; STEP_TRY(step_gemm_launch(gw, leaf));
        }
        im2col_kernel<<<g1(npos * 64), 256, 0, leaf>>>(xin, BN, Tin, Tout, dil, W.xcat[i]);
        STEP_LAUNCH_CHECK("im2col");
        StepGemm gw = gemm_desc(64, 64, (int)npos, W.dpre[i], 1, 64, W.xcat[i], 64, 1, W.dwcat + i * 4096, 64);
        gw.accumulate = 2; gw.splitk = -1;
        gw.a_rowsum = W.dbcat + i * 64;
        gw.compute_bf16 = BF16; STEP_TRY(step_gemm_launch(gw, leaf));
        dx_next = dx;
    }
    *dx0 = dx_next;
    if (!adj_pieces) STEP_TRY(adj_piece(0, NL - 2, lane.fork()));
    return STEP_OK;
}

extern "C" int step_gwnet_backward(const float* hist, int B, int N, int Cin, const float* hidden_last, const StepGwnetParams* p,
                                   const float* saved, float* work, const float* dpred, const StepGwnetParams* grads,
                                   float* dadj, int dropout, void* aux_stream, void* leaf_stream, void* stream) {
    STEP_REQUIRE(hist && hidden_last && p && saved && work && dpred && grads && dadj, "gwnet_backward: null argument");
    STEP_REQUIRE(B > 0 && N > 0 && Cin >= 2, "gwnet_backward: bad sizes");
    hipStream_t st = (hipStream_t)stream;
    AuxLane lane(st, (hipStream_t)aux_stream);
    AuxLane leaves(st, leaf_stream ? (hipStream_t)leaf_stream : (hipStream_t)aux_stream, 64);
    Saved S = carve_saved((float*)saved, B, N, dropout != 0);
    Work W = carve_work(work, B, N, true);
    const long BN = (long)B * N;
    const int allbf16 = p->gemm_bf16;
    auto split_for = [](long) { return -1; };

    STEP_TRY(pack_weights(p, W, st));
    STEP_TRY(zero(W.dwcat, (long)((float*)W.acc64 - W.dwcat) + 2L * NL * NCOPY * 64, st));
    const long NN = (long)N * N;

    {
        StepGemm g = gemm_desc(N, CE, OUT, dpred, 1, N, p->end2_w, CE, 1, W.d_e1, CE);
        g.batch = B; g.sab = (long)OUT * N; g.scb = (long)N * CE;
        STEP_TRY(step_gemm_launch(g, st));
        relu_bwd_kernel<<<g1(BN * CE), 256, 0, st>>>(W.d_e1, S.e1, BN * CE);
        StepGemm gx = gemm_desc((int)BN, CS, CE, W.d_e1, CE, 1, p->end1_w, CS, 1, W.d_xh, CS);
        gx.compute_bf16 = allbf16; STEP_TRY(step_gemm_launch(gx, st));
        relu_bwd_kernel<<<g1(BN * CS), 256, 0, st>>>(W.d_xh, S.xh, BN * CS);
        {
            hipStream_t leaf = leaves.fork();
            StepGemm gz = gemm_desc((int)BN, CS, CS, W.d_xh, CS, 1, W.wskip, CS, 1, W.dskip, CS);
            gz.compute_bf16 = allbf16; STEP_TRY(step_gemm_launch(gz, st));
            {
                StepGemm gw = gemm_desc(OUT, CE, N, dpred, N, 1, S.e1, CE, 1, grads->end2_w, CE);
                gw.batch = B; gw.sab = (long)OUT * N; gw.sbb = (long)N * CE; gw.scb = 0; gw.accumulate = 2;
                STEP_TRY(step_gemm_launch(gw, leaf));
                rowsum_mod_kernel<<<B * OUT, 256, 0, leaf>>>(dpred, N, OUT, grads->end2_b);
                STEP_LAUNCH_CHECK("end2_bias_grad");
                StepGemm gw1 = gemm_desc(CE, CS, (int)BN, W.d_e1, 1, CE, S.xh, CS, 1, grads->end1_w, CS);
                gw1.accumulate = 2; gw1.splitk = split_for(BN);
                gw1.a_rowsum = grads->end1_b;
                gw1.compute_bf16 = allbf16; STEP_TRY(step_gemm_launch(gw1, leaf));
            }
            STEP_TRY(zero(W.bsum, CS, leaf));
            STEP_TRY(step_colsum_launch(W.d_xh, BN, CS, CS, W.bsum, leaf));
            MPtr8 gb;
            for (int i = 0; i < NL; ++i) gb.p[i] = grads->skip_b[i];
            add_to8_kernel<<<1, 256, 0, leaf>>>(gb, W.bsum, CS);
            StepGemm gws = gemm_desc(CS, CS, (int)BN, W.d_xh, 1, CS, S.zlast, CS, 1, W.dwskip, CS);
            gws.accumulate = 2; gws.splitk = split_for(BN);
            gws.compute_bf16 = allbf16; STEP_TRY(step_gemm_launch(gws, leaf));
            if (hipMemcpyAsync(W.d_h2, W.d_xh, (size_t)BN * CS * sizeof(float), hipMemcpyDeviceToDevice, leaf) != hipSuccess) {
                step_set_error("gwnet_backward: copy failed");
                return STEP_ERR_HIP;
            }
            relu_bwd_kernel<<<g1(BN * CS), 256, 0, leaf>>>(W.d_h2, S.h2, BN * CS);
            StepGemm gw2 = gemm_desc(CS, CE, (int)BN, W.d_h2, 1, CS, S.h1, CE, 1, grads->fc_his2_w, CE);
            gw2.accumulate = 2; gw2.splitk = split_for(BN);
            gw2.a_rowsum = grads->fc_his2_b;
            gw2.compute_bf16 = allbf16; STEP_TRY(step_gemm_launch(gw2, leaf));
            StepGemm gh1 = gemm_desc((int)BN, CE, CS, W.d_h2, CS, 1, p->fc_his2_w, CE, 1, W.d_h1, CE);
            gh1.compute_bf16 = allbf16; STEP_TRY(step_gemm_launch(gh1, leaf));
            relu_bwd_kernel<<<g1(BN * CE), 256, 0, leaf>>>(W.d_h1, S.h1, BN * CE);
            StepGemm gw0 = gemm_desc(CE, HID, (int)BN, W.d_h1, 1, CE, hidden_last, HID, 1, grads->fc_his0_w, HID);
            gw0.accumulate = 2; gw0.splitk = split_for(BN);
            gw0.a_rowsum = grads->fc_his0_b;
            gw0.compute_bf16 = allbf16; STEP_TRY(step_gemm_launch(gw0, leaf));
        }
    }

    float* dx0 = nullptr;
    hipEvent_t adj_done = nullptr;
    if (allbf16) STEP_TRY(gwnet_layers_backward<true>(p, grads, S, W, B, N, &dx0, st, lane, leaves, &adj_done));
    else STEP_TRY(gwnet_layers_backward<false>(p, grads, S, W, B, N, &dx0, st, lane, leaves, &adj_done));
    STEP_TRY(lane.wait_done(adj_done));
    static const bool tail_leaves = []() { const char* e = getenv("STEP_TAIL_LEAVES"); return !(e && e[0] == '0'); }();
    if (!tail_leaves) STEP_TRY(leaves.join());
    hipStream_t leaf = tail_leaves ? leaves.fork() : st;
    row_dot_kernel<<<(unsigned)BN, 256, 0, st>>>(W.dPstk, S.Pstk, N, W.rf);
    row_dot_kernel<<<(unsigned)BN, 256, 0, st>>>(W.dPstk + B * NN, S.Pstk + B * NN, N, W.rb);
    rw_bwd_kernel<<<dim3(cdiv(N, 32), cdiv(N, 32), B), 256, 0, st>>>(W.dPstk, W.dPstk + B * NN, N, S.rs, S.cs, W.rf, W.rb, dadj);
    STEP_LAUNCH_CHECK("rw_bwd");
    {
        GatePtrs gg;
        SkipPtrs sg;
        for (int i = 0; i < NL; ++i) {
            gg.wf[i] = grads->filter_w[i]; gg.bf[i] = grads->filter_b[i]; gg.wg[i] = grads->gate_w[i]; gg.bg[i] = grads->gate_b[i];
            sg.w[i] = grads->skip_w[i]; sg.b[i] = nullptr;
        }
        start_conv_bwd_kernel<<<128, 256, 0, leaf>>>(hist, B, N, Cin, dx0, grads->start_w, grads->start_b);
        STEP_LAUNCH_CHECK("start_conv_bwd");
        unpack_gate_grad_kernel<<<dim3(16, NL), 256, 0, leaf>>>(W.dwcat, W.dbcat, gg);
        unpack_skip_grad_kernel<<<CS, CS, 0, leaf>>>(W.dwskip, sg);
    }
    {
        float* rdot = W.y7;
        sum_batches_kernel<<<g1(NN), 256, 0, leaf>>>(W.dPstk + 2 * B * NN, NN, B, W.dPa);
        row_dot_kernel<<<N, 256, 0, leaf>>>(W.dPa, S.Pa, N, rdot);
        softmax_relu_bwd_kernel<<<g1(NN), 256, 0, leaf>>>(S.Madp, S.Pa, W.dPa, rdot, N, W.dM);
        STEP_LAUNCH_CHECK("adp_bwd");
        StepGemm g1_ = gemm_desc(N, 10, N, W.dM, N, 1, p->nodevec2, 1, N, grads->nodevec1, 10);
        g1_.accumulate = 1;
        STEP_TRY(step_gemm_launch(g1_, leaf));
        StepGemm g2_ = gemm_desc(10, N, N, p->nodevec1, 1, 10, W.dM, N, 1, grads->nodevec2, N);
        g2_.accumulate = 1;
        STEP_TRY(step_gemm_launch(g2_, leaf));
    }
    STEP_LAUNCH_CHECK("rw_bwd");
    return STEP_OK;
}
```

step_amd/csrc/optim.hip:

```cpp
#include "common.h"
#include "step_internal.h"

namespace {

constexpr int NB = 1024;

__global__ __launch_bounds__(256) void sumsq_partial_kernel(const float* __restrict__ g, long n, float* __restrict__ partial) {
    __shared__ float red[4];
    float s = 0.f;
    const long n4 = n / 4;
    const float4* g4 = (const float4*)g;
    for (long i = (long)blockIdx.x * 256 + threadIdx.x; i < n4; i += (long)gridDim.x * 256) {
        float4 v = g4[i];
        s += v.x * v.x + v.y * v.y + v.z * v.z + v.w * v.w;
    }
    if (blockIdx.x == 0)
        for (long i = n4 * 4 + threadIdx.x; i < n; i += 256) s += g[i] * g[i];
    s = wave_sum(s);
    if ((threadIdx.x & 63) == 0) red[threadIdx.x >> 6] = s;
    __syncthreads();
    if (threadIdx.x == 0) partial[blockIdx.x] = red[0] + red[1] + red[2] + red[3];
}

__global__ __launch_bounds__(256) void adam_clip_kernel(float* __restrict__ p, const float* __restrict__ g, float* __restrict__ m,
// ... 17 lines not shown
        __syncthreads();
        if (threadIdx.x == 0) {
            const bool given = max_norm < 0.f;
            const float mx = given ? -max_norm : max_norm;
            const float norm = sqrtf(given ? *extra_sumsq : red[0] + red[1] + red[2] + red[3] + (extra_sumsq ? *extra_sumsq : 0.f));
            float c = mx > 0.f ? mx / (norm + 1e-6f) : 1.f;
            s_coef = c < 1.f ? c : 1.f;
            if (out_norm && blockIdx.x == 0) *out_norm = norm;
        }
        __syncthreads();
    }
    const float coef = s_coef;
    const float step_size = lr / bc1;
    for (long i = (long)blockIdx.x * 256 + threadIdx.x; i < n; i += (long)gridDim.x * 256) {
        const float pi = p[i];
        const float gi = g[i] * coef + wd * pi;
        const float mi = beta1 * m[i] + (1.f - beta1) * gi;
        const float vi = beta2 * v[i] + (1.f - beta2) * gi * gi;
        m[i] = mi; v[i] = vi;
        p[i] = pi - step_size * mi / (sqrtf(vi) / bc2_sqrt + eps);
    }
}

}

extern "C" long step_adam_work_floats(void) { return NB + 8; }

extern "C" int step_adam_clip(float* params, const float* grads, float* exp_avg, float* exp_avg_sq, long n, float lr, float beta1,
                              float beta2, float eps, float weight_decay, int step, float max_norm, float* work, float* out_norm,
                              void* stream) {
    return step_adam_clip_sharded(params, grads, exp_avg, exp_avg_sq, n, lr, beta1, beta2, eps, weight_decay, step, max_norm, nullptr, work,
                                  out_norm, stream);
}

static int adam_clip_launch(float* params, const float* grads, float* exp_avg, float* exp_avg_sq, long n, float lr, float beta1,
                            float beta2, float eps, float weight_decay, int step, float max_norm, const float* extra_sumsq,
                            float* work, float* out_norm, const StepDynState* dyn, void* stream);
extern "C" int step_adam_clip_sharded(float* params, const float* grads, float* exp_avg, float* exp_avg_sq, long n, float lr, float beta1,
                                      float beta2, float eps, float weight_decay, int step, float max_norm, const float* extra_sumsq,
                                      float* work, float* out_norm, void* stream) {
    return adam_clip_launch(params, grads, exp_avg, exp_avg_sq, n, lr, beta1, beta2, eps, weight_decay, step, max_norm, extra_sumsq, work, out_norm,
                            nullptr, stream);
}
extern "C" int step_adam_clip_dyn(float* params, const float* grads, float* exp_avg, float* exp_avg_sq, long n, float beta1, float beta2,
                                  float eps, float weight_decay, float max_norm, const float* extra_sumsq, float* work, float* out_norm,
                                  const StepDynState* dyn, void* stream) {
    STEP_REQUIRE(dyn, "adam_clip_dyn: null state");
    return adam_clip_launch(params, grads, exp_avg, exp_avg_sq, n, 0.f, beta1, beta2, eps, weight_decay, 1, max_norm, extra_sumsq, work, out_norm, dyn,
                            stream);
}
__global__ void dyn_advance_kernel(StepDynState* s) {
    uint64_t z = s->seed_xor + 0x9E3779B97F4A7C15ull;
    z = (z ^ (z >> 30)) * 0xBF58476D1CE4E5B9ull;
    z = (z ^ (z >> 27)) * 0x94D049BB133111EBull;
    s->seed_xor = z ^ (z >> 31);
    s->adam_step += 1;
}
extern "C" int step_dyn_advance(StepDynState* dyn, void* stream) {
    STEP_REQUIRE(dyn, "dyn_advance: null state");
    dyn_advance_kernel<<<1, 1, 0, (hipStream_t)stream>>>(dyn);
    STEP_LAUNCH_CHECK("dyn_advance");
    return STEP_OK;
}
static int adam_clip_launch(float* params, const float* grads, float* exp_avg, float* exp_avg_sq, long n, float lr, float beta1,
                            float beta2, float eps, float weight_decay, int step, float max_norm, const float* extra_sumsq,
                            float* work, float* out_norm, const StepDynState* dyn, void* stream) {
    STEP_REQUIRE(params && grads && exp_avg && exp_avg_sq && work && n > 0 && step >= 1, "adam_clip: bad arguments");
    STEP_REQUIRE((((uintptr_t)grads) & 15) == 0, "adam_clip: gradient buffer must be 16-byte aligned");
    STEP_REQUIRE(max_norm >= 0.f || extra_sumsq, "adam_clip: max_norm < 0 (squared norm supplied by the caller) needs extra_sumsq");
    hipStream_t st = (hipStream_t)stream;
    sumsq_partial_kernel<<<NB, 256, 0, st>>>(grads, n, work);
    STEP_LAUNCH_CHECK("sumsq_partial");
    const float bc1 = 1.f - powf(beta1, (float)step);
    const float bc2 = 1.f - powf(beta2, (float)step);
    int blocks = (int)((n + 255) / 256);
    if (blocks > 4096) blocks = 4096;
    adam_clip_kernel<<<blocks, 256, 0, st>>>(params, grads, exp_avg, exp_avg_sq, n, lr, beta1, beta2, eps, weight_decay, bc1, sqrtf(bc2),
                                             max_norm, work, NB, extra_sumsq, out_norm, dyn);
    STEP_LAUNCH_CHECK("adam_clip");
    return STEP_OK;
}

namespace {
__global__ __launch_bounds__(256) void loss_reduce_kernel(const float* __restrict__ pred, const float* __restrict__ real, long n1, long rs,
                                                          float scale, float shift,
                                                          const float* __restrict__ theta, const float* __restrict__ prior, long n2,
                                                          float null_val, double* __restrict__ acc ) {
    __shared__ double red[4][3];
    double s_abs = 0.0, s_cnt = 0.0, s_bce = 0.0;
    const long stride = (long)gridDim.x * 256;
    for (long i = (long)blockIdx.x * 256 + threadIdx.x; i < n1; i += stride) {
        const float y = real[i * rs] * scale + shift;
        if (fabsf(y - null_val) > 5e-5f) { s_abs += fabsf((pred[i] * scale + shift) - y); s_cnt += 1.0; }
    }
    for (long i = (long)blockIdx.x * 256 + threadIdx.x; i < n2; i += stride) {
        const float t = theta[i], y = prior[i];
        const float l1 = fmaxf(logf(t), -100.f), l0 = fmaxf(logf(1.f - t), -100.f);
        s_bce -= (double)(y * l1 + (1.f - y) * l0);
    }
    for (int o = 32; o > 0; o >>= 1) {
        s_abs += __shfl_xor(s_abs, o, 64); s_cnt += __shfl_xor(s_cnt, o, 64); s_bce += __shfl_xor(s_bce, o, 64);
    }
    if ((threadIdx.x & 63) == 0) { red[threadIdx.x >> 6][0] = s_abs; red[threadIdx.x >> 6][1] = s_cnt; red[threadIdx.x >> 6][2] = s_bce; }
    __syncthreads();
    if (threadIdx.x < 3) atomicAdd(&acc[threadIdx.x], red[0][threadIdx.x] + red[1][threadIdx.x] + red[2][threadIdx.x] + red[3][threadIdx.x]);
}
__global__ __launch_bounds__(256) void loss_finish_kernel(const float* __restrict__ pred, const float* __restrict__ real, long n1, long rs,
                                                          float scale, float shift,
                                                          const float* __restrict__ theta, const float* __restrict__ prior, long n2,
                                                          float null_val, float coef, const double* __restrict__ acc,
                                                          float* __restrict__ loss, float* __restrict__ dpred, float* __restrict__ dtheta,
                                                          const StepDynState* __restrict__ dyn) {
    if (dyn) coef = dyn->gsl_coef;
    const double cnt = acc[1];
    const float inv_cnt = cnt > 0.0 ? (float)(1.0 / cnt) : 0.f;
    if (blockIdx.x == 0 && threadIdx.x == 0)
        *loss = (cnt > 0.0 ? (float)(acc[0] / cnt) : 0.f) + coef * (float)(acc[2] / (double)n2);
    const long stride = (long)gridDim.x * 256;
    for (long i = (long)blockIdx.x * 256 + threadIdx.x; i < n1; i += stride) {
        const float y = real[i * rs] * scale + shift, d = (pred[i] * scale + shift) - y;
        const float m = fabsf(y - null_val) > 5e-5f ? inv_cnt * scale : 0.f;
        dpred[i] = d > 0.f ? m : (d < 0.f ? -m : 0.f);
    }
    const float sc = coef / (float)n2;
    for (long i = (long)blockIdx.x * 256 + threadIdx.x; i < n2; i += stride) {
        const float t = theta[i], y = prior[i];
        dtheta[i] = sc * (t - y) / fmaxf(t * (1.f - t), 1e-12f);
    }
}
__global__ __launch_bounds__(256) void scale2_kernel(const float* __restrict__ a, long na, const float* __restrict__ b, long nb,
                                                     const float* __restrict__ g, float* __restrict__ oa, float* __restrict__ ob) {
    const float s = *g;
    const long stride = (long)gridDim.x * 256;
    for (long i = (long)blockIdx.x * 256 + threadIdx.x; i < na; i += stride) oa[i] = a[i] * s;
    for (long i = (long)blockIdx.x * 256 + threadIdx.x; i < nb; i += stride) ob[i] = b[i] * s;
}
}

static int loss_launch(const float* pred, const float* real, long n_pred, long real_stride, float scale, float shift, const float* theta,
                       const float* prior, long n_adj, float null_val, float coef, double* work, float* loss, float* dpred, float* dtheta,
                       const StepDynState* dyn, void* stream);
extern "C" int step_loss_scaled_fwd_bwd(const float* pred, const float* real, long n_pred, long real_stride, float scale, float shift,
                                        const float* theta, const float* prior, long n_adj, float null_val, float coef,
                                        double* work , float* loss, float* dpred, float* dtheta, void* stream) {
    return loss_launch(pred, real, n_pred, real_stride, scale, shift, theta, prior, n_adj, null_val, coef, work, loss, dpred, dtheta, nullptr, stream);
}
extern "C" int step_loss_scaled_fwd_bwd_dyn(const float* pred, const float* real, long n_pred, long real_stride, float scale, float shift,
                                            const float* theta, const float* prior, long n_adj, float null_val, double* work, float* loss,
                                            float* dpred, float* dtheta, const StepDynState* dyn, void* stream) {
    STEP_REQUIRE(dyn, "step_loss_dyn: null state");
    return loss_launch(pred, real, n_pred, real_stride, scale, shift, theta, prior, n_adj, null_val, 0.f, work, loss, dpred, dtheta, dyn, stream);
}
static int loss_launch(const float* pred, const float* real, long n_pred, long real_stride, float scale, float shift, const float* theta,
                       const float* prior, long n_adj, float null_val, float coef, double* work, float* loss, float* dpred, float* dtheta,
                       const StepDynState* dyn, void* stream) {
    STEP_REQUIRE(pred && real && theta && prior && work && loss && dpred && dtheta && n_pred > 0 && n_adj > 0 && real_stride >= 1,
                 "step_loss: bad arguments");
    hipStream_t st = (hipStream_t)stream;
    if (hipMemsetAsync(work, 0, 3 * sizeof(double), st) != hipSuccess) { step_set_error("step_loss: memset failed"); return STEP_ERR_HIP; }
    long nmax = n_pred > n_adj ? n_pred : n_adj;
    int blocks = (int)((nmax + 255) / 256);
    if (blocks > 1024) blocks = 1024;
    int rblocks = (int)(nmax / 4096);
    rblocks = rblocks < 1 ? 1 : (rblocks > 1024 ? 1024 : rblocks);
    loss_reduce_kernel<<<rblocks, 256, 0, st>>>(pred, real, n_pred, real_stride, scale, shift, theta, prior, n_adj, null_val, work);
    STEP_LAUNCH_CHECK("loss_reduce");
    loss_finish_kernel<<<blocks, 256, 0, st>>>(pred, real, n_pred, real_stride, scale, shift, theta, prior, n_adj, null_val, coef, work, loss,
                                               dpred, dtheta, dyn);
    STEP_LAUNCH_CHECK("loss_finish");
    return STEP_OK;
}
extern "C" int step_loss_fwd_bwd(const float* pred, const float* real, long n_pred, const float* theta, const float* prior, long n_adj,
                                 float null_val, float coef, double* work , float* loss, float* dpred, float* dtheta,
                                 void* stream) {
    return step_loss_scaled_fwd_bwd(pred, real, n_pred, 1, 1.f, 0.f, theta, prior, n_adj, null_val, coef, work, loss, dpred, dtheta, stream);
}
namespace {
__global__ __launch_bounds__(256) void masked_metrics_kernel(const float* __restrict__ pred, long ps, const float* __restrict__ real, long rs, long n,
                                                             float null_val, double* __restrict__ work, float* __restrict__ out) {
    __shared__ double red[4][5];
    __shared__ bool last;
    double a[5] = {0.0, 0.0, 0.0, 0.0, 0.0};
    const long stride = (long)gridDim.x * 256;
    for (long i = (long)blockIdx.x * 256 + threadIdx.x; i < n; i += stride) {
        const float p = pred[i * ps], y = real[i * rs];
        if (fabsf(y - null_val) > 5e-5f) { const float d = p - y; a[0] += fabsf(d); a[1] += (double)d * d; a[2] += 1.0; }
        const float y0 = fabsf(y) < 1e-4f ? 0.f : y;
        if (fabsf(y0) > 5e-5f) { a[3] += fabsf(fabsf(p - y0) / y0); a[4] += 1.0; }
    }
#pragma unroll
    for (int k = 0; k < 5; ++k)
        for (int o = 32; o > 0; o >>= 1) a[k] += __shfl_xor(a[k], o, 64);
    if ((threadIdx.x & 63) == 0)
        for (int k = 0; k < 5; ++k) red[threadIdx.x >> 6][k] = a[k];
    __syncthreads();
    if (threadIdx.x < 5) atomicAdd(&work[threadIdx.x], red[0][threadIdx.x] + red[1][threadIdx.x] + red[2][threadIdx.x] + red[3][threadIdx.x]);
    __threadfence();
    __syncthreads();
    if (threadIdx.x == 0) last = atomicAdd((unsigned int*)(work + 5), 1u) == gridDim.x - 1;
    __syncthreads();
    if (last && threadIdx.x == 0) {
        __threadfence();
        volatile double* w = work;
        const double s_abs = w[0], s_sq = w[1], cnt = w[2], s_ape = w[3], cnt0 = w[4];
        out[0] = cnt > 0.0 ? (float)(s_abs / cnt) : 0.f;
        out[1] = cnt > 0.0 ? sqrtf((float)(s_sq / cnt)) : 0.f;
        out[2] = cnt0 > 0.0 ? (float)(s_ape / cnt0) : 0.f;
        for (int k = 0; k < 6; ++k) w[k] = 0.0;
    }
}
}
extern "C" int step_masked_metrics(const float* pred, long pred_stride, const float* real, long real_stride, long n, float null_val,
                                   double* work , float* out , void* stream) {
    STEP_REQUIRE(pred && real && work && out && n > 0 && pred_stride >= 1 && real_stride >= 1, "step_masked_metrics: bad arguments");
    int blocks = (int)(n / 4096);
    blocks = blocks < 1 ? 1 : (blocks > 256 ? 256 : blocks);
    masked_metrics_kernel<<<blocks, 256, 0, (hipStream_t)stream>>>(pred, pred_stride, real, real_stride, n, null_val, work, out);
    STEP_LAUNCH_CHECK("masked_metrics");
    return STEP_OK;
}
extern "C" int step_scale2(const float* a, long na, const float* b, long nb, const float* g, float* out_a, float* out_b, void* stream) {
    STEP_REQUIRE(a && b && g && out_a && out_b && na > 0 && nb > 0, "step_scale2: bad arguments");
    long nmax = na > nb ? na : nb;
    int blocks = (int)((nmax + 255) / 256);
    if (blocks > 1024) blocks = 1024;
    scale2_kernel<<<blocks, 256, 0, (hipStream_t)stream>>>(a, na, b, nb, g, out_a, out_b);
    STEP_LAUNCH_CHECK("scale2");
    return STEP_OK;
}
```

step_amd/csrc/step_internal.h:

```cpp
#pragma once
#include <hip/hip_runtime.h>
#include <vector>
#include "../../include/step_hip.h"

enum { GEMM_FUSED_INTERLEAVED = 1, GEMM_FUSED_FFN_FWD = 2, GEMM_FUSED_MASKNZ = 4, GEMM_FUSED_BF16OUT = 8 };
struct GemmFused {
    const float* dotw; float* dots;
    const float* bnx; const float* bncoef; const float* bnstat;
    int channels, period;
    int flags;
    const float* ffn_bias; const void* maskx; float p; unsigned seed_lo, seed_hi, site;
};

struct GemmKSeg { long a_off, b_off, a_bs, b_bs; int a_rs, b_rs; };
constexpr int GEMM_KSEG_MAX = 128;
int step_gemm_segmented_launch(StepGemm g, const GemmKSeg* ktab, int ktab_per, hipStream_t st);

int step_gemm_launch(StepGemm g, hipStream_t st);
int step_gemm_auto_splitk(int M, int N, int K, int batch);
int step_gemm_launch_fused(StepGemm g, const GemmFused& fused, hipStream_t st);
int step_gemm_bf16_launch(StepGemm g, hipStream_t st, const GemmFused* fused = nullptr);
int step_gemm_f32_fast_launch(StepGemm g, hipStream_t st, const GemmFused* fused = nullptr);

static inline StepGemm gemm_desc(int M, int N, int K, const float* A, long sam, long sak, const float* B, long sbk,
                                 long sbn, float* C, long ldc) {
    StepGemm g;
    memset(&g, 0, sizeof(g));
    g.M = M; g.N = N; g.K = K; g.batch = 1;
    g.A = A; g.sam = sam; g.sak = sak;
    g.B = B; g.sbk = sbk; g.sbn = sbn;
    g.C = C; g.ldc = ldc; g.scn = 1;
    g.alpha = 1.f; g.splitk = 1;
    return g;
}

int step_gemm_rowsum_separate(StepGemm* g, hipStream_t st);
int dgl_conv2_fwd_mfma(const float* a1, const float* w, const float* b, const float* sc, const float* sh, float* a2, float* partial,
                       int N, int T1, int* nblk, hipStream_t st);
int dgl_conv2_dgrad_mfma(const float* dz, const float* w, float* din, int N, int T1, const float* bnx, const float* coef, const float* stat,
                         int own, hipStream_t st);
int dgl_conv2_wgrad_xhat_mfma(const float* dz, const float* a1, const float* stat1, float* scratch, float* graw, int N, int T1, hipStream_t st);
int dgl_conv2_wgrad_finish(const float* graw, const float* w, const float* stat1, const float* gamma1, const float* beta1, double count,
                           float* dw, float* db, float* dgamma1, float* dbeta1, float* coef1, int raw, hipStream_t st);
int dgl_conv1_fwd_cl(const float* x, const float* w, const float* b, void* a1h, float* partial, int N, int T, int stat_limit, int* nblk,
                     hipStream_t st);
long dgl_conv2_pack_floats();
int dgl_conv2_fwd_cl(const void* a1h, const float* w, const float* b, const float* sc, const float* sh, void* a2h, float* partial, int N,
                     int T1, int* nblk, float* pack, hipStream_t st);
int dgl_conv2_dgrad_cl(const void* dz2h, const float* w, const float* sc, void* dz1h, int N, int T1, const void* a1h, const float* coef,
                       const float* stat, int own, float* pack, hipStream_t st);
int dgl_conv2_wgrad_cl(const void* dz2h, const void* a1h, float* scratch, float* graw, int N, int T1, hipStream_t st);
int dgl_conv1_wgrad_cl(const void* dz1h, const float* x, float* scratch, float* dw, float* db, int N, int T, hipStream_t st);
long dgl_conv2_wgrad_scratch_floats(int N, int T1);
int dgl_conv2_wgrad_mfma(const float* dz, const float* a1, const float* sc, const float* sh, float* scratch, float* dw, float* db, int N,
                         int T1, hipStream_t st);
int dgl_conv1_wgrad_mfma(const float* dz, const float* x, float* scratch, float* dw, float* db, int N, int T, hipStream_t st);
int step_colsum_launch(const float* x, long rows, int cols, long ld, float* out, hipStream_t st);

struct AuxLane {
    hipStream_t main, aux;
    bool on;
    int next = 0, base = 0;
    AuxLane(hipStream_t m, hipStream_t a, int base_ = 0) : main(m), aux(a), on(a != nullptr && a != m), base(base_) {}
    static hipEvent_t event(int k) {
        thread_local std::vector<hipEvent_t> pool[16];
        int dev = 0;
        (void)hipGetDevice(&dev);
        std::vector<hipEvent_t>& v = pool[dev & 15];
        while ((int)v.size() <= k) {
            hipEvent_t e;
            if (hipEventCreateWithFlags(&e, hipEventDisableTiming) != hipSuccess) return nullptr;
            v.push_back(e);
        }
        return v[k];
    }
    hipStream_t fork() {
        if (!on) return main;
        hipEvent_t e = event(base + (next++ & 63));
        if (!e || hipEventRecord(e, main) != hipSuccess || hipStreamWaitEvent(aux, e, 0) != hipSuccess) { on = false; return main; }
        return aux;
    }
    hipEvent_t mark() {
        if (!on) return nullptr;
        hipEvent_t e = event(base + (next++ & 63));
        if (!e || hipEventRecord(e, main) != hipSuccess) { on = false; return nullptr; }
        return e;
    }
    hipStream_t after(hipEvent_t e) {
        if (!on || !e) return main;
        if (hipStreamWaitEvent(aux, e, 0) != hipSuccess) { on = false; return main; }
        return aux;
    }
    hipEvent_t done() {
        if (!on) return nullptr;
        hipEvent_t e = event(base + (next++ & 63));
        if (!e || hipEventRecord(e, aux) != hipSuccess) return nullptr;
        return e;
    }
    int wait_done(hipEvent_t e) {
        if (!on) return STEP_OK;
        if (!e) return join();
        if (hipStreamWaitEvent(main, e, 0) != hipSuccess) { step_set_error("backward: stream join failed"); return STEP_ERR_HIP; }
        return STEP_OK;
    }
    int join() {
        if (!on) return STEP_OK;
        hipEvent_t e = event(base + (next++ & 63));
        if (!e || hipEventRecord(e, aux) != hipSuccess || hipStreamWaitEvent(main, e, 0) != hipSuccess) {
            step_set_error("backward: stream join failed");
            return STEP_ERR_HIP;
        }
        return STEP_OK;
    }
};
```

step_amd/step_arch/step.py:

```python
import ctypes
import os

import torch
from torch import nn

from .. import _lib
from .tsformer import TSFormer
from .graphwavenet import GraphWaveNet, fill_gwnet_struct
from .discrete_graph_learning import DiscreteGraphLearning, fill_dgl_struct
from . import eval_cache as _ec

TEMPERATURE = 0.5
BN_MOMENTUM = 0.1


def _f32(n, device):
    return torch.empty(int(n), device=device, dtype=torch.float32)


class LongHistoryRef:

    def __init__(self, data, t0, length, channels=None, t0_host=None):
        assert data.is_cuda and data.dtype == torch.float32 and data.dim() == 3 and data.is_contiguous()
        assert t0.is_cuda and t0.dtype == torch.int64 and t0.dim() == 1
# ... 22 lines not shown
        full = slice(None)
        if isinstance(idx, tuple) and len(idx) == 4 and all(i == full for i in idx[:3] if isinstance(i, slice)) and all(isinstance(i, slice) for i in idx[:3]):
            sel = idx[3]
            if isinstance(sel, slice):
                sel = list(range(len(self.channels)))[sel]
            elif torch.is_tensor(sel):
                sel = sel.tolist()
            return LongHistoryRef(self.data, self.t0, self.length, [self.channels[int(c)] for c in sel], t0_host=self.t0_host)
        raise IndexError("LongHistoryRef supports the runner's feature selection only: ref[:, :, :, features]")


class DeviceWindowLoader:

    def __init__(self, data, long_len, horizon=12):
        self.data = data.contiguous().float()
        assert self.data.is_cuda
        self.long_len, self.horizon = int(long_len), int(horizon)

    def batch(self, t0, t0_host=None):
        if t0_host is None and not (torch.is_tensor(t0) and t0.is_cuda):
            t0_host = t0.tolist() if hasattr(t0, "tolist") else list(t0)
        t0 = torch.as_tensor(t0, dtype=torch.int64, device=self.data.device).contiguous()
        B, (T, N, C), H = t0.shape[0], self.data.shape, self.horizon
        hist = torch.empty(B, H, N, C, device=self.data.device)
        fut = torch.empty(B, H, N, C, device=self.data.device)
        _lib.call("step_gather_windows", _lib.ptr(self.data), T, N, C, 0, _lib.ptr(t0), B, 0, H, None, _lib.ptr(hist), _lib.ptr(fut),
                  _lib.stream())
        return hist, LongHistoryRef(self.data, t0, self.long_len, t0_host=t0_host), fut


class _StepFunction(torch.autograd.Function):

    @staticmethod
    def forward(ctx, model, hist, long_hist, u, *params):
        L = _lib
        dev = hist.device
        B, T12, N, Cin = hist.shape
        Lh = long_hist.shape[1]
        training = model.training
        st = L.stream()
        hist = hist.contiguous().float()
        frozen = model._take_prefetched(long_hist)
        ec_on, model._ec_on = model._ec_on, False
        ec = model._eval_cache_plan(long_hist, N, Lh // 12, dev) if ec_on else None
        dgl, be = model.discrete_graph_learning, model.backend
        sh = dgl._shard
        if sh is not None and not training:
            if dgl._slice_dirty:
                raise RuntimeError("evaluation of a time-sliced graph learner needs the gathered fc.weight: call "
                                   "model.discrete_graph_learning.gather_fc_weight() on ALL ranks after the training epoch "
                                   "(the runner's on_epoch_end) before the master-only validation")
            if torch.is_grad_enabled() and any(p.requires_grad for p in params):
                raise RuntimeError("a time-sliced graph learner evaluates without gradients only (wrap the call in torch.no_grad())")
            sh = None
        bf = {"f32": 0, "bf16": 1}[model.matmul_precision]
        dstruct, bstruct = model._param_structs(bf, full=sh is None)
        Ttr = dgl.train_length if sh is None else sh["Ts"]
        series_nt = dgl._series_nt if sh is None else dgl._series_slice
        drop = be.dropout if training else 0.0
        g_key = model._eval_g_key(bf, N, Ttr) if ec_on else None
        g = model._eval_g_lookup(g_key) if g_key is not None else None
        g_kept = g is not None
        if g_kept:
            gsaved = gwork = None
        else:
            gsaved = _f32(L.lib().step_dgl_global_saved_floats(N, Ttr), dev)
            gwork = _f32(L.lib().step_dgl_global_work_floats(N, Ttr, 0), dev)
            g = _f32(N * 100, dev).view(N, 100)
        esaved = _f32(L.lib().step_dgl_edges_saved_floats(B, N), dev)
        to = int(L.lib().step_dgl_edges_theta_offset(N))
        theta = esaved[to:to + B * N * N].view(B, N, N)
        adj = _f32(B * N * N, dev).view(B, N, N)
        wsaved = _f32(L.lib().step_gwnet_saved_floats(B, N, int(drop > 0)), dev)
        wwork = _f32(L.lib().step_gwnet_work_floats(B, N, 0), dev)
        pred = _f32(B * 12 * N, dev).view(B, 12, N)
        seed, seed_gw = model._next_seed(), model._next_seed()
        side = model._side_stream(dev) if model.overlap_streams else None
        main = torch.cuda.current_stream()
        if side is not None:
            ready = torch.cuda.Event()
            ready.record(main)
        P = Lh // 12
        prep_done = None
        if side is not None and model.split_wavenet_prep and model._dyn is None:
            prep = model._side_stream(dev, "aux")
            prep.wait_event(ready)
            with torch.cuda.stream(prep):
                hist.record_stream(prep)
                L.call("step_gwnet_forward_phase_dyn", L.ptr(hist), B, N, Cin, None, None, ctypes.byref(bstruct),
                       int(training) | (2 if (training and model.track_dead_bn7) else 0),
                       float(drop), seed_gw, BN_MOMENTUM, L.ptr(wsaved), L.ptr(wwork), None, 5, None, L.stream())
                prep_done = torch.cuda.Event()
                prep_done.record(prep)

        def graph_and_layers(sst):
            if g_kept:
                pass
            elif sh is None:
                L.call("step_dgl_global_forward", L.ptr(series_nt), N, Ttr, ctypes.byref(dstruct), int(training), BN_MOMENTUM,
                       L.ptr(gsaved), L.ptr(gwork), L.ptr(g), sst)
            else:
                sstruct = dgl.shard_struct()
                sums = torch.zeros(48, dtype=torch.float64, device=dev)
                go = L.lib().step_dgl_global_offset(N, Ttr, 2)
                exchange = {1: sums[:16], 2: sums[16:], 3: gsaved[go:go + N * 100]}
                for phase in (1, 2, 3, 4):
                    L.call("step_dgl_global_forward_shard", L.ptr(series_nt), N, Ttr, ctypes.byref(dstruct), int(training), BN_MOMENTUM,
                           L.ptr(gsaved), L.ptr(gwork), L.ptr(sums), L.ptr(g), ctypes.byref(sstruct), phase, sst)
                    if phase in exchange:
                        model._sum_over_ranks(exchange[phase])
            L.call("step_dgl_edges_forward_dyn", L.ptr(g), N, B, ctypes.byref(dstruct), L.ptr(u) if u is not None else None, seed,
                   TEMPERATURE, L.ptr(esaved), L.ptr(theta), L.ptr(adj), L.ptr(model._dyn), sst)
            if prep_done is not None:
                torch.cuda.current_stream().wait_event(prep_done)
            L.call("step_gwnet_forward_phase_dyn", L.ptr(hist), B, N, Cin, None, L.ptr(adj), ctypes.byref(bstruct),
                   int(training) | (2 if (training and model.track_dead_bn7) else 0),
                   float(drop), seed_gw, BN_MOMENTUM, L.ptr(wsaved), L.ptr(wwork), None, 6 if prep_done is not None else 1, L.ptr(model._dyn), sst)
            if training:
                with torch.no_grad():
                    torch._foreach_add_([m.num_batches_tracked for m in (dgl.bn1, dgl.bn2, dgl.bn3, *list(be.bn)[:8 if model.track_dead_bn7 else 7])], 1)

        if frozen is None and ec is not None and ec["hit"]:
            frozen = model._eval_cache_load(ec, B, N, dev)
        if frozen is None:
            ks = model._side_stream(dev, "knn") if (side is not None and os.environ.get("STEP_KNN_STREAM", "0") == "1") else None
            frozen = model._frozen_branch(long_hist, B, N, knn_stream=ks)
        if side is not None:
            side.wait_event(ready)
            try:
                with torch.cuda.stream(side):
                    hist.record_stream(side)
                    if u is not None:
                        u.record_stream(side)
                    graph_and_layers(L.stream())
            except BaseException:
                main.wait_stream(side)
                raise
        else:
            graph_and_layers(st)
        if frozen["done"] is not None:
            main.wait_event(frozen["done"])
        enc, sim, adj_knn = frozen["enc"], frozen["sim"], frozen["adj_knn"]
        try:
            L.call("step_gwnet_forward_phase", L.ptr(hist), B, N, Cin, L.ptr(enc["last"]), None, ctypes.byref(bstruct), int(training),
                   float(drop), seed_gw, BN_MOMENTUM, L.ptr(wsaved), L.ptr(wwork), None, 3, st)
        finally:
            if side is not None:
                main.wait_stream(side)
        L.call("step_gwnet_forward_phase", L.ptr(hist), B, N, Cin, None, None, ctypes.byref(bstruct), int(training),
               float(drop), seed_gw, BN_MOMENTUM, L.ptr(wsaved), L.ptr(wwork), L.ptr(pred), 4, st)
        if frozen.get("knn_done") is not None:
            main.wait_event(frozen["knn_done"])
        if ec is not None:
            model._eval_cache_store(ec, frozen, B, N, dev)
        if g_key is not None and not g_kept:
            model._eval_g = (g_key, g)
        ctx.model = model
        ctx.dims = (B, N, Cin, Ttr, float(drop))
        ctx.held = (hist, enc["last"], g, gsaved, esaved, wsaved)
        ctx.esaved_version = esaved._version
        ctx.mark_non_differentiable(adj_knn)
        model._last = {"sampled_adj": adj, "sim": sim, "hidden_bf16": enc["hidden_bf16"], "saved_gwnet": wsaved, "g": g,
                       "hidden_last": enc["last"]}
        return pred.unsqueeze(-1), theta, adj_knn

    @staticmethod
    def backward(ctx, dpred, dtheta, _dknn):
        L = _lib
        model = ctx.model
        B, N, Cin, Ttr, drop = ctx.dims
        hist, last, g, gsaved, esaved, wsaved = ctx.held
        dev = hist.device
        st = L.stream()
        be, dgl = model.backend, model.discrete_graph_learning
        layout = model._grad_layout()
        fo, fn, _ = layout["items"]["dgl.fc_w"]
        flat, views, gw_grads, dg_grads = model._grad_buffers(layout, dev)
        flat[:fo].zero_()
        if fo + fn < layout["total"]:
            flat[fo + fn:].zero_()
        bf = {"f32": 0, "bf16": 1}[model.matmul_precision]
        dstruct, bstruct = model._param_structs(bf, full=False)
        dpred = dpred.contiguous().float().view(B, 12, N) if dpred is not None else torch.zeros(B, 12, N, device=dev)
        dadj = _f32(B * N * N, dev)
        wwork = _f32(L.lib().step_gwnet_work_floats(B, N, 1), dev)
        use_aux = model.overlap_streams and os.environ.get("STEP_NO_AUX", "0") != "1"
        aux = ctypes.c_void_p(model._side_stream(dev, "aux").cuda_stream) if use_aux else None
        leaf = ctypes.c_void_p(model._side_stream(dev, "leaf").cuda_stream) if (use_aux and os.environ.get("STEP_LEAF_STREAM", "0") == "1") else None
        joined = [False]

        def join_aux():
            if aux is not None:
                torch.cuda.current_stream().wait_stream(model._side_stream(dev, "aux"))
            if leaf is not None:
                torch.cuda.current_stream().wait_stream(model._side_stream(dev, "leaf"))
            joined[0] = True
        if esaved._version != ctx.esaved_version:
            raise RuntimeError("step_amd.STEP: the returned edge probabilities (theta) were modified in place after forward(); the native "
                               "backward reads that buffer -- use an out-of-place op (theta.clamp(...)) or theta.clone()")
        FRESH = 16
        try:
            L.call("step_gwnet_backward", L.ptr(hist), B, N, Cin, L.ptr(last), ctypes.byref(bstruct), L.ptr(wsaved), L.ptr(wwork),
                   L.ptr(dpred), ctypes.byref(gw_grads), L.ptr(dadj), int(drop > 0), aux, leaf, st)
            ework = _f32(L.lib().step_dgl_edges_work_floats(N), dev)
            dgv = _f32(N * 100, dev)
            dth = dtheta.contiguous().float() if dtheta is not None else None
            L.call("step_dgl_edges_backward", L.ptr(g), N, B, ctypes.byref(dstruct), L.ptr(esaved), L.ptr(dth) if dth is not None else None,
                   L.ptr(dadj), TEMPERATURE, L.ptr(ework), ctypes.byref(dg_grads), L.ptr(dgv), leaf if leaf is not None else aux, st)
            gwork = _f32(L.lib().step_dgl_global_work_floats(N, Ttr, 1), dev)
            fo, fn, _ = layout["items"]["dgl.fc_w"]
            assert fo + fn == layout["total"] or fo + ((fn + 3) & ~3) == layout["total"]
            assert layout["norm_slot"] == fo - 4
            sh = dgl._shard
            if sh is None:
                L.call("step_dgl_global_backward_phase", L.ptr(dgl._series_nt), N, Ttr, ctypes.byref(dstruct), L.ptr(gsaved), L.ptr(dgv),
                       L.ptr(gwork), ctypes.byref(dg_grads), 1 | FRESH, st)
                pending = model._reduce_begin(flat[fo:fo + fn])
                L.call("step_dgl_global_backward_phase", L.ptr(dgl._series_nt), N, Ttr, ctypes.byref(dstruct), L.ptr(gsaved), L.ptr(dgv),
                       L.ptr(gwork), ctypes.byref(dg_grads), 2, st)
                join_aux()
                pending += model._reduce_begin(flat[:fo])
                model._reduce_finish(flat, pending, flat)
# ... 18 lines not shown
                torch.mul(own.square(), float(world), out=flat[ns:ns + 1])
                model._reduce_finish(flat, model._reduce_begin(flat[:fo]), flat[:fo])
                model._other_slices_sumsq = torch.addcmul(flat[ns:ns + 1], own, own, value=-1.0)
                slices = flat[ns:ns + 1].clone()
                flat[ns:ns + 1].zero_()
                rep = torch.linalg.vector_norm(flat[:fo])
                model._total_sumsq = torch.addcmul(slices, rep, rep)
        finally:
            if not joined[0]:
                join_aux()
        del wwork, ework
        model._flat_grad = flat
        model._backward_count = getattr(model, "_backward_count", 0) + 1
        model._drop_eval_g()
        ctx.held = None
        del views, gw_grads, dg_grads
        if model.flat_gradients_only:
            return (None, None, None, None) + (None,) * len(layout["order"])
        return (None, None, None, None) + tuple(flat[o:o + n].view(shape) for o, n, shape in (layout["items"][k] for k in layout["order"]))


_STREAMS = {}


def _concurrent_stream(dev, tries=8, priority=0):
    if os.environ.get("STEP_STREAM_PROBE", "1") == "0":
        return torch.cuda.Stream(device=dev, priority=priority)
    main = torch.cuda.current_stream(dev)
    mine = [(n, v) for (n, t, i), v in _STREAMS.items() if t == dev.type and i == dev.index]
    kept, flag = [], ctypes.c_int(0)

    def overlaps(a, b):
        _lib.call("step_streams_concurrent", ctypes.c_void_p(a.cuda_stream), ctypes.c_void_p(b.cuda_stream), ctypes.byref(flag))
        return bool(flag.value)
    best, best_score = None, -1
    full = 100 + 10 * sum(1 for n, _ in mine if n == "prefetch") + sum(1 for n, _ in mine if n != "prefetch")
    for _ in range(tries):
        s = torch.cuda.Stream(device=dev, priority=priority)
        kept.append(s)
        score = 0
        if overlaps(main, s):
            score = 100
            for n, o in mine:
                if overlaps(o, s):
                    score += 10 if n == "prefetch" else 1
        if score > best_score:
            best, best_score = s, score
        if score >= full:
            break
    return best


class STEP(nn.Module):

    def __init__(self, dataset_name, pre_trained_tsformer_path, tsformer_args, backend_args, dgl_args):
        super().__init__()
        self.dataset_name = dataset_name
        self.pre_trained_tsformer_path = pre_trained_tsformer_path
        self.tsformer = TSFormer(**tsformer_args)
        self.backend = GraphWaveNet(**backend_args)
        self.load_pre_trained_model()
        self.discrete_graph_learning = DiscreteGraphLearning(**dgl_args)
        self.gumbel_noise = "device"
        self.matmul_precision = "f32"
        self.track_dead_bn7 = False
        self._noise_override = None
        self._seed_ctr = 0
        self._dyn = None
        self._process_group = None
        self._struct_cache = {}
        self._bwd_cache = None
        self._trainable_cache = None
        self.flat_gradients_only = False
        self._comm = None
        self._min_world = 1
        self._layout = None
        self._zg_params = None
        self._zg_key = None
        self._last = {}
        self._flat_param = None
        self._flat_grad = None
        self._backward_count = 0
        self.overlap_streams = os.environ.get("STEP_NO_OVERLAP", "0") != "1"
        self.split_wavenet_prep = os.environ.get("STEP_PREP_SPLIT", "0") == "1"
        self.prefetch_knn_stream = os.environ.get("STEP_PREFETCH_KNN_STREAM", "0") == "1"
        self._prefetched = None
        self._precision_override = None
        self.prefetch_fifo = 2
        self._alias = {}
        self.prefetch_enabled = os.environ.get("STEP_NO_PREFETCH", "0") != "1"
        self._reduce_wait_ms = None
        self._reduce_events = []
        self._small_events = []
        self.eval_cache_bytes = 0
        self._eval_cache_chunk_windows = 256
        self.eval_cache_stats = _ec.new_stats()
        self._eval_cache = None
        self._eval_cache_alloc = None
        self._eval_g = None
        self._ec_on = False

    def load_pre_trained_model(self):
        if self.pre_trained_tsformer_path is not None:
            ckpt = torch.load(self.pre_trained_tsformer_path, map_location="cpu")
            self.tsformer.load_state_dict(ckpt["model_state_dict"])
        for p in self.tsformer.parameters():
            p.requires_grad = False
        if "_eval_cache" in self.__dict__:
            self._invalidate_eval_cache()

    def _side_stream(self, dev, name="side"):
        key = (name, dev.type, dev.index)
        if key not in _STREAMS:
            _STREAMS[key] = _concurrent_stream(dev, priority=int(os.environ.get("STEP_PRIORITY_" + name.upper(), "0")))
        return _STREAMS[key]

    def _frozen_branch(self, long_hist, B, N, knn_stream=None, channel=0):
        L = _lib
        st = L.stream()
        dev = self.backend.nodevec1.device
        Lh = long_hist.shape[1]
        series = _f32(B * N * Lh, dev).view(B * N, Lh)
        if isinstance(long_hist, LongHistoryRef):
            d = long_hist.data
            L.call("step_gather_windows", L.ptr(d), d.shape[0], d.shape[1], d.shape[2], long_hist.channels[channel], L.ptr(long_hist.t0), B, Lh, 12,
                   L.ptr(series), None, None, st)
        else:
            long_hist = long_hist.contiguous().float()
            L.call("step_pack_long_history", L.ptr(long_hist), B, Lh, N, long_hist.shape[3], int(channel), L.ptr(series), st)
        P = Lh // 12
        tie = self._eval_cache_tie(N, P) if (self.eval_cache_bytes > 0 and not self.training) else None
        enc = self.tsformer.encode_series(series)
        if tie is not None and self._eval_cache_tie(N, P) != tie:
            tie = None
        sim = _f32(B * N * N, dev).view(B, N, N)
        adj_knn = _f32(B * N * N, dev).view(B, N, N)
        kwork = torch.empty(L.lib().step_knn_workspace_bytes(B, N, P * 96), dtype=torch.uint8, device=dev)
        knn_done = None
        if knn_stream is not None:
            enc_done = torch.cuda.Event()
            enc_done.record()
            knn_stream.wait_event(enc_done)
            with torch.cuda.stream(knn_stream):
                for t in (enc["hidden_bf16"], enc["sqnorm"], sim, adj_knn, kwork):
                    t.record_stream(knn_stream)
                L.call("step_knn_graph", L.ptr(enc["hidden_bf16"]), L.ptr(enc["sqnorm"]), B, N, P * 96, self.discrete_graph_learning.k * N,
                       L.ptr(sim), L.ptr(adj_knn), L.ptr(kwork), kwork.numel(), L.stream())
                knn_done = torch.cuda.Event()
                knn_done.record()
        else:
            L.call("step_knn_graph", L.ptr(enc["hidden_bf16"]), L.ptr(enc["sqnorm"]), B, N, P * 96, self.discrete_graph_learning.k * N,
                   L.ptr(sim), L.ptr(adj_knn), L.ptr(kwork), kwork.numel(), st)
        return {"enc": enc, "sim": sim, "adj_knn": adj_knn, "held": (series, kwork, long_hist), "done": None, "knn_done": knn_done, "tie": tie}

    @staticmethod
    def _batch_key(long_hist, channel=0):
        if isinstance(long_hist, LongHistoryRef):
            t = long_hist.t0
            return (t.data_ptr(), tuple(long_hist.shape[:3]), t._version, True, long_hist.channels[channel])
        return (long_hist.data_ptr(), tuple(long_hist.shape[:3]), long_hist._version, False, int(channel))

    def alias_batch(self, source, derived, channel=0):
        if len(self._alias) > 8:
            self._alias.clear()
        self._alias[self._batch_key(derived, 0)] = self._batch_key(source, channel)

    def prefetch(self, long_history_data, channel=0):
# ... 444 lines not shown
```

step_amd/step_loss.py:

```python
import ctypes

import numpy as np
import torch


def masked_mae(preds, labels, null_val=np.nan):
    if np.isnan(null_val):
        mask = ~torch.isnan(labels)
    else:
        mask = (labels - null_val).abs() > 5e-5
    mask = mask.float()
    mask = mask / torch.mean(mask)
    mask = torch.nan_to_num(mask, nan=0.0)
    loss = torch.abs(preds - labels) * mask
    return torch.mean(torch.nan_to_num(loss, nan=0.0))


def _flat_stride(x):
    if x.is_contiguous():
        return 1
    if x.dim() < 2 or x.shape[-1] != 1:
        return None
    s = x.stride(-2)
    exp = s
    for d in range(x.dim() - 2, -1, -1):
        if x.shape[d] != 1 and x.stride(d) != exp:
            return None
        exp *= x.shape[d]
    return s


class _NativeStepLoss(torch.autograd.Function):

    @staticmethod
    def forward(ctx, prediction, real_value, theta, priori_adj, coef, null_val, scale, shift):
        from . import _lib
        p = prediction.contiguous().float()
        r = real_value.float()
        rs = _flat_stride(r)
        if rs is None:
            r, rs = r.contiguous(), 1
        t = theta.contiguous().float()
        a = priori_adj.contiguous().float()
        loss = torch.empty((), device=p.device, dtype=torch.float32)
        dp, dt = torch.empty_like(p), torch.empty_like(t)
        work = torch.empty(3, device=p.device, dtype=torch.float64)
        assert r.is_cuda and r.dtype == torch.float32
        if torch.is_tensor(coef):
            _lib.call("step_loss_scaled_fwd_bwd_dyn", _lib.ptr(p), ctypes.c_void_p(r.data_ptr()), p.numel(), rs, float(scale), float(shift), _lib.ptr(t),
                      _lib.ptr(a), t.numel(), float(null_val), _lib.ptr(work), _lib.ptr(loss), _lib.ptr(dp), _lib.ptr(dt), _lib.ptr(coef), _lib.stream())
        else:
            _lib.call("step_loss_scaled_fwd_bwd", _lib.ptr(p), ctypes.c_void_p(r.data_ptr()), p.numel(), rs, float(scale), float(shift), _lib.ptr(t),
                      _lib.ptr(a), t.numel(), float(null_val), float(coef), _lib.ptr(work), _lib.ptr(loss), _lib.ptr(dp), _lib.ptr(dt), _lib.stream())
        ctx.save_for_backward(dp, dt)
        ctx.shapes = (prediction.shape, theta.shape)
        return loss

    @staticmethod
    def backward(ctx, g):
        from . import _lib
        dp, dt = ctx.saved_tensors
        if g.is_cuda and g.dtype == torch.float32 and g.numel() == 1:
            op, ot = torch.empty_like(dp), torch.empty_like(dt)
            _lib.call("step_scale2", _lib.ptr(dp), dp.numel(), _lib.ptr(dt), dt.numel(), _lib.ptr(g.contiguous()), _lib.ptr(op), _lib.ptr(ot),
                      _lib.stream())
        else:
            op, ot = dp * g, dt * g
        return op.view(ctx.shapes[0]), None, ot.view(ctx.shapes[1]), None, None, None, None, None


def step_loss_native(prediction, real_value, theta, priori_adj, gsl_coefficient, null_val=0.0, rescale=None, horizons=None):
    if horizons is not None:
        return train_tail(prediction, real_value, theta, priori_adj, gsl_coefficient, null_val=null_val, rescale=rescale, horizons=horizons)[0]
    mean, std = (0.0, 1.0) if rescale is None else rescale
    return _NativeStepLoss.apply(prediction, real_value, theta, priori_adj, gsl_coefficient, null_val, std, mean)


def _bhn_strides(x):
    st = x.stride()[:3]
    return tuple(int(v) for v in st) if all(v >= 1 for v in st) else None


_TAIL_WORK = {}


def _tail_work(device):
    from . import _lib
    key = (device.index, torch.cuda.current_stream().cuda_stream)
    w = _TAIL_WORK.get(key)
    if w is None:
        w = _TAIL_WORK[key] = torch.zeros(_lib.lib().step_train_tail_work_doubles(), dtype=torch.float64, device=device)
    return w


class _TrainTail(torch.autograd.Function):

    @staticmethod
    def forward(ctx, prediction, real_value, theta, priori_adj, coef, null_val, scale, shift, k):
        from . import _lib
        B, H, N = prediction.shape[:3]
        p, r = prediction.detach(), real_value.detach()
        ps, rs = _bhn_strides(p), _bhn_strides(r)
        if ps is None:
            p = p.contiguous()
            ps = _bhn_strides(p)
        if rs is None:
            r = r.contiguous()
            rs = _bhn_strides(r)
        t = theta.detach().contiguous()
        a = priori_adj.detach().contiguous().float()
        dev = p.device
        loss = torch.empty((), device=dev, dtype=torch.float32)
        metrics = torch.empty(3, device=dev, dtype=torch.float32)
        dp = torch.empty((B, H, N), device=dev, dtype=torch.float32)
        dt = torch.empty_like(t)
        _lib.call("step_train_tail", ctypes.c_void_p(p.data_ptr()), *ps, ctypes.c_void_p(r.data_ptr()), *rs, B, H, N, int(k), float(scale),
                  float(shift), float(null_val), _lib.ptr(t), _lib.ptr(a), t.numel(), float(coef), _lib.ptr(_tail_work(dev)), _lib.ptr(loss),
                  _lib.ptr(metrics), _lib.ptr(dp), _lib.ptr(dt), _lib.stream())
        ctx.save_for_backward(dp, dt)
        ctx.shapes = (prediction.shape, theta.shape)
        ctx.mark_non_differentiable(metrics)
        ctx.set_materialize_grads(False)
        return loss, metrics

    @staticmethod
    def backward(ctx, g, _g_metrics):
        from . import _lib
        if g is None:
            return (None,) * 9
        dp, dt = ctx.saved_tensors
        if g.is_cuda and g.dtype == torch.float32 and g.numel() == 1:
            op, ot = torch.empty_like(dp), torch.empty_like(dt)
            _lib.call("step_scale2", _lib.ptr(dp), dp.numel(), _lib.ptr(dt), dt.numel(), _lib.ptr(g.contiguous()), _lib.ptr(op), _lib.ptr(ot),
                      _lib.stream())
        else:
            op, ot = dp * g, dt * g
# ... 64 lines not shown
```

Measured before the change: 2358.

## Fold memsets and bf16 conversions into producer kernels; enable wavenet prep split

Several small memsets are folded into neighbouring kernels: BN finalize kernels clear the shiftdot buffer, the bn3 backward kernel zeroes dots_o, and the loss reduction uses a ring buffer that is reset in-kernel instead of a memset each step. The rw_build and replicate_adp kernels now write bf16 copies of the transition matrices directly, which removes a separate stacks_to_bf16 pass. The wavenet prep phase becomes on by default and runs on the main stream when prefetched, with the BN counter updates moved accordingly. The aim is fewer launches and less redundant memory traffic, at the cost of more complex kernel contracts and new environment-gated paths.

```diff
diff --git a/include/step_hip.h b/include/step_hip.h
--- a/include/step_hip.h
+++ b/include/step_hip.h
@@ -119,6 +119,7 @@
 int step_gwnet_backward(const float* hist, int B, int N, int Cin, const float* hidden_last, const StepGwnetParams* p,
                         const float* saved, float* work, const float* dpred, const StepGwnetParams* grads,
                         float* dadj, int dropout, void* aux_stream, void* leaf_stream, void* stream);
+int step_selftest_row_dots(const float* dP, const float* P, int N, long rows, float* rf, float* rb, int folded, void* stream);
 
 int step_pt_dropout(const float* x, float* y, long n, float p, uint64_t seed, uint32_t site, void* stream);
 int step_pt_ffn_hidden_fwd(const float* x, const float* w1, const float* b1, long R, float p, uint64_t seed, uint32_t site,
@@ -196,6 +197,10 @@
 int step_loss_scaled_fwd_bwd(const float* pred, const float* real, long n_pred, long real_stride, float scale, float shift,
                              const float* theta, const float* prior, long n_adj, float null_val, float coef, double* work, float* loss,
                              float* dpred, float* dtheta, void* stream);
+long step_loss_ring_doubles(void);
+int step_loss_ring_fwd_bwd(const float* pred, const float* real, long n_pred, long real_stride, float scale, float shift,
+                           const float* theta, const float* prior, long n_adj, float null_val, float coef, double* ring, float* loss,
+                           float* dpred, float* dtheta, void* stream);
 int step_masked_metrics(const float* pred, long pred_stride, const float* real, long real_stride, long n, float null_val, double* work,
                         float* out, void* stream);
 int step_scale2(const float* a, long na, const float* b, long nb, const float* g, float* out_a, float* out_b, void* stream);
diff --git a/step_amd/_lib.py b/step_amd/_lib.py
--- a/step_amd/_lib.py
+++ b/step_amd/_lib.py
@@ -86,6 +86,7 @@
     "step_gwnet_forward": (_i, [_vp, _i, _i, _i, _vp, _vp, _PG, _i, _f, _u64, _f, _vp, _vp, _vp, _vp]),
     "step_gwnet_forward_phase": (_i, [_vp, _i, _i, _i, _vp, _vp, _PG, _i, _f, _u64, _f, _vp, _vp, _vp, _i, _vp]),
     "step_gwnet_backward": (_i, [_vp, _i, _i, _i, _vp, _PG, _vp, _vp, _vp, _PG, _vp, _i, _vp, _vp, _vp]),
+    "step_selftest_row_dots": (_i, [_vp, _vp, _i, _l, _vp, _vp, _i, _vp]),
     "step_pt_dropout": (_i, [_vp, _vp, _l, _f, _u64, ctypes.c_uint32, _vp]),
     "step_pt_ffn_hidden_fwd": (_i, [_vp, _vp, _vp, _l, _f, _u64, ctypes.c_uint32, _vp, _vp]),
     "step_pt_ffn_hidden_bwd": (_i, [_vp, _vp, _vp, _l, _f, _vp, _vp]),
@@ -129,6 +130,8 @@
     "step_colsum": (_i, [_vp, _l, _i, _l, _vp, _vp]),
     "step_loss_fwd_bwd": (_i, [_vp, _vp, _l, _vp, _vp, _l, _f, _f, _vp, _vp, _vp, _vp, _vp]),
     "step_loss_scaled_fwd_bwd": (_i, [_vp, _vp, _l, _l, _f, _f, _vp, _vp, _l, _f, _f, _vp, _vp, _vp, _vp, _vp]),
+    "step_loss_ring_doubles": (_l, []),
+    "step_loss_ring_fwd_bwd": (_i, [_vp, _vp, _l, _l, _f, _f, _vp, _vp, _l, _f, _f, _vp, _vp, _vp, _vp, _vp]),
     "step_scale2": (_i, [_vp, _l, _vp, _l, _vp, _vp, _vp, _vp]),
     "step_masked_metrics": (_i, [_vp, _l, _vp, _l, _l, _f, _vp, _vp, _vp]),
     "step_adam_work_floats": (_l, []),
diff --git a/step_amd/csrc/dgl.hip b/step_amd/csrc/dgl.hip
--- a/step_amd/csrc/dgl.hip
+++ b/step_amd/csrc/dgl.hip
@@ -74,9 +74,10 @@
 __global__ __launch_bounds__(256) void bn_finalize_kernel(const float* __restrict__ partial, int nblk, int C, double count,
                                                           const float* __restrict__ gamma, const float* __restrict__ beta,
                                                           float* __restrict__ rmean, float* __restrict__ rvar, int training,
-                                                          float momentum, float* __restrict__ stat) {
+                                                          float momentum, float* __restrict__ stat, float* __restrict__ clear128) {
     __shared__ double r1[256], r2[256];
     const int c = blockIdx.x, tid = threadIdx.x;
+    if (clear128 && c == 0 && tid < 128) clear128[tid] = 0.f;
     double mean, var;
     if (training) {
         double a = 0.0, q = 0.0;
@@ -136,8 +137,10 @@
 }
 __global__ void bn_finalize_sums_kernel(const double* __restrict__ sums, int C, double count, const float* __restrict__ gamma,
                                         const float* __restrict__ beta, float* __restrict__ rmean, float* __restrict__ rvar,
-                                        int training, float momentum, float* __restrict__ stat) {
+                                        int training, float momentum, float* __restrict__ stat, float* __restrict__ clear128 = nullptr) {
     const int c = threadIdx.x;
+    if (clear128)
+        for (int i = c; i < 128; i += blockDim.x) clear128[i] = 0.f;
     if (c >= C) return;
     double mean, var;
     if (training) {
@@ -194,9 +197,11 @@
                                                            const float* __restrict__ gamma, const float* __restrict__ stat,
                                                            float* __restrict__ dgamma, float* __restrict__ dbeta,
                                                            float* __restrict__ dbias, float* __restrict__ dgpre,
-                                                           float* __restrict__ dgpreT, float* __restrict__ colsum) {
+                                                           float* __restrict__ dgpreT, float* __restrict__ colsum,
+                                                           float* __restrict__ clear_dots_o = nullptr) {
     __shared__ double r1[256], r2[256];
     const int j = blockIdx.x, tid = threadIdx.x;
+    if (clear_dots_o && tid < 32) clear_dots_o[j * 32 + tid] = 0.f;
     const float mean = stat[2 * EMB + j], rstd = stat[3 * EMB + j];
     double a = 0.0, q = 0.0;
     for (int n = tid; n < N; n += 256) {
@@ -721,13 +726,13 @@
 }
 
 static int dgl_bn_stats(const float* partial, int nblk, int C, double count, const float* gamma, const float* beta, float* rm, float* rv,
-                        int training, float momentum, float* stat, double* sums, hipStream_t st) {
+                        int training, float momentum, float* stat, double* sums, hipStream_t st, float* clear128 = nullptr) {
     if (nblk < 8192) {
-        bn_finalize_kernel<<<C, 256, 0, st>>>(partial, nblk, C, count, gamma, beta, rm, rv, training, momentum, stat);
+        bn_finalize_kernel<<<C, 256, 0, st>>>(partial, nblk, C, count, gamma, beta, rm, rv, training, momentum, stat, clear128);
     } else {
         if (hipMemsetAsync(sums, 0, 2 * C * sizeof(double), st) != hipSuccess) { step_set_error("memset failed"); return STEP_ERR_HIP; }
         bn_sums_sliced_kernel<<<dim3(C, 32), 256, 0, st>>>(partial, nblk, C, sums);
-        bn_finalize_sums_kernel<<<1, 64, 0, st>>>(sums, C, count, gamma, beta, rm, rv, training, momentum, stat);
+        bn_finalize_sums_kernel<<<1, 64, 0, st>>>(sums, C, count, gamma, beta, rm, rv, training, momentum, stat, clear128);
     }
     STEP_LAUNCH_CHECK("bn_stats");
     return STEP_OK;
@@ -747,6 +752,7 @@
     double* own_sums = (double*)(work + part_floats + dgl_conv2_pack_floats());
     float* wp = saved_wp(saved, N, T);
     float* shiftdot = wp + (long)EMB * 16 * T2;
+    float* const clear_shiftdot = (cl && step_chain_folds()) ? shiftdot : nullptr;
     if (all || phase == 1) {
         int nblk;
         if (cl) {
@@ -777,15 +783,18 @@
             nblk = grid.x * grid.y;
         }
         if (shard) bn_sums_kernel<<<16, 256, 0, st>>>(partial, nblk, 16, sums + 16);
-        else STEP_TRY(dgl_bn_stats(partial, nblk, 16, count2, p->bn2_w, p->bn2_b, p->bn2_rm, p->bn2_rv, training, momentum, st2, own_sums, st));
+        else STEP_TRY(dgl_bn_stats(partial, nblk, 16, count2, p->bn2_w, p->bn2_b, p->bn2_rm, p->bn2_rv, training, momentum, st2, own_sums, st,
+                                   all ? clear_shiftdot : nullptr));
         STEP_LAUNCH_CHECK("bn2");
     }
     if (all || phase == 3) {
-        if (shard) bn_finalize_sums_kernel<<<1, 64, 0, st>>>(sums + 16, 16, count2, p->bn2_w, p->bn2_b, p->bn2_rm, p->bn2_rv, training, momentum, st2);
+        if (shard) bn_finalize_sums_kernel<<<1, 64, 0, st>>>(sums + 16, 16, count2, p->bn2_w, p->bn2_b, p->bn2_rm, p->bn2_rv, training, momentum, st2,
+                                                             clear_shiftdot);
+        const bool shift_cleared = clear_shiftdot && (shard || all);
         const long K = 16L * T2;
         StepGemm gm = gemm_desc(N, EMB, (int)K, a2, K, 1, p->fc_w, 1, K, gpre, EMB);
         if (cl) {
-            if (hipMemsetAsync(shiftdot, 0, 128 * sizeof(float), st) != hipSuccess) { step_set_error("memset failed"); return STEP_ERR_HIP; }
+            if (!shift_cleared && hipMemsetAsync(shiftdot, 0, 128 * sizeof(float), st) != hipSuccess) { step_set_error("memset failed"); return STEP_ERR_HIP; }
             fc_prep_kernel<<<dim3(cdiv(T2, 256), EMB), 256, 0, st>>>(p->fc_w, st2, (uint4*)wp, shiftdot, T2);
             gpre_init_kernel<<<cdiv((long)N * EMB, 256), 256, 0, st>>>(gpre, shiftdot, (long)N * EMB);
             STEP_LAUNCH_CHECK("fc_prep");
@@ -891,14 +900,16 @@
         const float* wp = saved_wp((float*)saved, N, T);
         float* dots_o = coef + 256 + 64 + 1344;
         float* colsum = coef + 128;
+        const bool folds = step_chain_folds();
         if (do_fc) {
-            bn3_relu_bwd_kernel<<<EMB, 256, 0, st>>>(dg, gpre, N, p->bn3_w, st3, grads->bn3_w, grads->bn3_b, grads->fc_b, dgpre, dgpreT, colsum);
+            bn3_relu_bwd_kernel<<<EMB, 256, 0, st>>>(dg, gpre, N, p->bn3_w, st3, grads->bn3_w, grads->bn3_b, grads->fc_b, dgpre, dgpreT, colsum,
+                                                     folds ? dots_o : nullptr);
             STEP_LAUNCH_CHECK("bn3_bwd");
             StepGemm gm = gemm_desc(EMB, (int)K, N, dgpre, 1, EMB, a2, K, 1, wraw, K);
             gm.b_bf16 = 1;
             gm.compute_bf16 = 1;
             STEP_TRY(step_gemm_launch(gm, st));
-            if (hipMemsetAsync(dots_o, 0, EMB * 32 * sizeof(float), st) != hipSuccess) { step_set_error("memset failed"); return STEP_ERR_HIP; }
+            if (!folds && hipMemsetAsync(dots_o, 0, EMB * 32 * sizeof(float), st) != hipSuccess) { step_set_error("memset failed"); return STEP_ERR_HIP; }
             fc_unpermute_kernel<<<dim3(cdiv(T2, 256), EMB), 256, 0, st>>>(wraw, p->fc_w, st2, colsum, grads->fc_w, dots_o, T2, fresh_fc);
             dots_reduce_kernel<<<1, 64, 0, st>>>(dots_o, dots);
             STEP_LAUNCH_CHECK("fc_unpermute");
diff --git a/step_amd/csrc/gwnet.hip b/step_amd/csrc/gwnet.hip
--- a/step_amd/csrc/gwnet.hip
+++ b/step_amd/csrc/gwnet.hip
@@ -76,21 +76,33 @@
     __syncthreads();
     if (w == 0 && j < N) atomicAdd(&cs[(long)b * N + j], red[0][threadIdx.x] + red[1][threadIdx.x] + red[2][threadIdx.x] + red[3][threadIdx.x]);
 }
+__device__ __forceinline__ uint16_t bf16_bits(float v) {
+    typedef __attribute__((ext_vector_type(2))) float f2;
+    typedef __attribute__((ext_vector_type(2))) __bf16 b2;
+    f2 t = {v, 0.f};
+    return (uint16_t)(__builtin_bit_cast(uint32_t, __builtin_convertvector(t, b2)) & 0xffffu);
+}
 __global__ __launch_bounds__(256) void rw_build_kernel(const float* __restrict__ A, int N, const float* __restrict__ rs,
                                                        const float* __restrict__ cs, float* __restrict__ Pf, float* __restrict__ Pb,
-                                                       float* __restrict__ PfT, float* __restrict__ PbT) {
+                                                       float* __restrict__ PfT, float* __restrict__ PbT, int N8,
+                                                       uint16_t* __restrict__ P16, uint16_t* __restrict__ PT16) {
     __shared__ float tile[32][33];
     const int b = blockIdx.z, i0 = blockIdx.y * 32, j0 = blockIdx.x * 32;
     const int tx = threadIdx.x & 31, ty = threadIdx.x >> 5;
     const long base = (long)b * N * N;
+    const long base16 = (long)b * N * N8, slot16 = (long)gridDim.z * N * N8;
     for (int r = ty; r < 32; r += 8) {
         int i = i0 + r, j = j0 + tx;
         float a = (i < N && j < N) ? A[base + (long)i * N + j] : 0.f;
         tile[r][tx] = a;
         if (i < N && j < N) {
             const float v = a + (i == j ? 1.f : 0.f);
-            Pf[base + (long)i * N + j] = v / rs[(long)b * N + i];
-            PbT[base + (long)i * N + j] = v / cs[(long)b * N + j];
+            const float pf = v / rs[(long)b * N + i], pbt = v / cs[(long)b * N + j];
+            Pf[base + (long)i * N + j] = pf;
+            PbT[base + (long)i * N + j] = pbt;
+            if (P16) { P16[base16 + (long)i * N8 + j] = bf16_bits(pf); PT16[slot16 + base16 + (long)i * N8 + j] = bf16_bits(pbt); }
+        } else if (P16 && i < N && j < N8) {
+            P16[base16 + (long)i * N8 + j] = 0; PT16[slot16 + base16 + (long)i * N8 + j] = 0;
         }
     }
     __syncthreads();
@@ -98,17 +110,30 @@
         int j = j0 + r, i = i0 + tx;
         if (i < N && j < N) {
             const float v = tile[tx][r] + (i == j ? 1.f : 0.f);
-            Pb[base + (long)j * N + i] = v / cs[(long)b * N + j];
-            PfT[base + (long)j * N + i] = v / rs[(long)b * N + i];
-        }
-    }
-}
-__global__ void replicate_adp_kernel(const float* __restrict__ Pa, int N, int B, float* __restrict__ P2, float* __restrict__ PT2) {
+            const float pb = v / cs[(long)b * N + j], pft = v / rs[(long)b * N + i];
+            Pb[base + (long)j * N + i] = pb;
+            PfT[base + (long)j * N + i] = pft;
+            if (P16) { P16[slot16 + base16 + (long)j * N8 + i] = bf16_bits(pb); PT16[base16 + (long)j * N8 + i] = bf16_bits(pft); }
+        } else if (P16 && j < N && i < N8) {
+            P16[slot16 + base16 + (long)j * N8 + i] = 0; PT16[base16 + (long)j * N8 + i] = 0;
+        }
+    }
+}
+__global__ void replicate_adp_kernel(const float* __restrict__ Pa, int N, int B, float* __restrict__ P2, float* __restrict__ PT2, int N8,
+                                     uint16_t* __restrict__ P16_2, uint16_t* __restrict__ PT16_2) {
     long idx = (long)blockIdx.x * 256 + threadIdx.x;
     if (idx >= (long)N * N) return;
     int i = idx / N, j = idx % N;
     float v = Pa[idx], vt = Pa[(long)j * N + i];
     for (int b = 0; b < B; ++b) { P2[(long)b * N * N + idx] = v; PT2[(long)b * N * N + idx] = vt; }
+    if (!P16_2) return;
+    const uint16_t h = bf16_bits(v), ht = bf16_bits(vt);
+    for (int b = 0; b < B; ++b) {
+        const long row = ((long)b * N + i) * N8;
+        P16_2[row + j] = h; PT16_2[row + j] = ht;
+        if (j == N - 1)
+            for (int k = N; k < N8; ++k) { P16_2[row + k] = 0; PT16_2[row + k] = 0; }
+    }
 }
 __global__ void stacks_to_bf16_kernel(const float* __restrict__ P, const float* __restrict__ PT, long rows, int N, int N8,
                                       uint16_t* __restrict__ P16, uint16_t* __restrict__ PT16) {
@@ -160,6 +185,20 @@
     if ((threadIdx.x & 63) == 0) red[threadIdx.x >> 6] = s;
     __syncthreads();
     if (threadIdx.x == 0) out[row] = red[0] + red[1] + red[2] + red[3];
+}
+__global__ __launch_bounds__(256) void row_dot2_kernel(const float* __restrict__ dP, const float* __restrict__ P, int N, long rows,
+                                                       float* __restrict__ out0, float* __restrict__ out1) {
+    __shared__ float red[4];
+    const long row = blockIdx.x;
+    float s = 0.f;
+    for (int j = threadIdx.x; j < N; j += 256) s += dP[row * N + j] * P[row * N + j];
+    s = wave_sum(s);
+    if ((threadIdx.x & 63) == 0) red[threadIdx.x >> 6] = s;
+    __syncthreads();
+    if (threadIdx.x == 0) {
+        const float d = red[0] + red[1] + red[2] + red[3];
+        if (row < rows) out0[row] = d; else out1[row - rows] = d;
+    }
 }
 __global__ __launch_bounds__(256) void rw_bwd_kernel(const float* __restrict__ dPf, const float* __restrict__ dPb, int N,
                                                      const float* __restrict__ rs, const float* __restrict__ cs,
@@ -930,7 +969,10 @@
             StepGemm g = gemm_desc(N, N, 10, p->nodevec1, 10, 1, p->nodevec2, N, 1, S.Madp, N);
             STEP_TRY(step_gemm_launch(g, st));
             softmax_relu_rows_kernel<<<N, 256, 0, st>>>(S.Madp, N, S.Pa);
-            replicate_adp_kernel<<<g1(NN), 256, 0, st>>>(S.Pa, N, B, S.Pstk + 2 * B * NN, S.PTstk + 2 * B * NN);
+            const bool fold16 = p->gemm_bf16 && step_chain_folds();
+            const long NN8 = (long)N * n8(N);
+            replicate_adp_kernel<<<g1(NN), 256, 0, st>>>(S.Pa, N, B, S.Pstk + 2 * B * NN, S.PTstk + 2 * B * NN, n8(N),
+                                                         fold16 ? S.P16 + 2 * B * NN8 : nullptr, fold16 ? S.PT16 + 2 * B * NN8 : nullptr);
             STEP_LAUNCH_CHECK("adp_softmax");
         }
         STEP_TRY(pack_weights(p, W, st));
@@ -945,10 +987,12 @@
             if (slices < 1) slices = 1;
             col_sums_kernel<<<dim3(cdiv(N, 64), slices, B), 256, 0, st>>>(adj, N, S.cs);
         }
+        const bool fold16 = p->gemm_bf16 && step_chain_folds();
         rw_build_kernel<<<dim3(cdiv(N, 32), cdiv(N, 32), B), 256, 0, st>>>(adj, N, S.rs, S.cs, S.Pstk, S.Pstk + B * NN, S.PTstk,
-                                                                           S.PTstk + B * NN);
+                                                                           S.PTstk + B * NN, n8(N), fold16 ? S.P16 : nullptr,
+                                                                           fold16 ? S.PT16 : nullptr);
         STEP_LAUNCH_CHECK("rw_build");
-        if (p->gemm_bf16) {
+        if (p->gemm_bf16 && !fold16) {
             const long rows = 3L * B * N;
             stacks_to_bf16_kernel<<<dim3((unsigned)cdiv(rows * (n8(N) / 2), 256), 2), 256, 0, st>>>(S.Pstk, S.PTstk, rows, N, n8(N), S.P16,
                                                                                                    S.PT16);
@@ -980,6 +1024,19 @@
         g4.bias = p->end2_b;
         g4.compute_bf16 = allbf16; STEP_TRY(step_gemm_launch(g4, st));
     }
+    return STEP_OK;
+}
+
+extern "C" int step_selftest_row_dots(const float* dP, const float* P, int N, long rows, float* rf, float* rb, int folded, void* stream) {
+    STEP_REQUIRE(dP && P && rf && rb && N > 0 && rows > 0 && 2 * rows <= 0x7fffffffL, "selftest_row_dots: bad arguments");
+    hipStream_t st = (hipStream_t)stream;
+    if (folded) {
+        row_dot2_kernel<<<(unsigned)(2 * rows), 256, 0, st>>>(dP, P, N, rows, rf, rb);
+    } else {
+        row_dot_kernel<<<(unsigned)rows, 256, 0, st>>>(dP, P, N, rf);
+        row_dot_kernel<<<(unsigned)rows, 256, 0, st>>>(dP + rows * N, P + rows * N, N, rb);
+    }
+    STEP_LAUNCH_CHECK("selftest_row_dots");
     return STEP_OK;
 }
 
@@ -1130,8 +1187,12 @@
     static const bool tail_leaves = []() { const char* e = getenv("STEP_TAIL_LEAVES"); return !(e && e[0] == '0'); }();
     if (!tail_leaves) STEP_TRY(leaves.join());
     hipStream_t leaf = tail_leaves ? leaves.fork() : st;
-    row_dot_kernel<<<(unsigned)BN, 256, 0, st>>>(W.dPstk, S.Pstk, N, W.rf);
-    row_dot_kernel<<<(unsigned)BN, 256, 0, st>>>(W.dPstk + B * NN, S.Pstk + B * NN, N, W.rb);
+    if (step_chain_folds()) {
+        row_dot2_kernel<<<(unsigned)(2 * BN), 256, 0, st>>>(W.dPstk, S.Pstk, N, BN, W.rf, W.rb);
+    } else {
+        row_dot_kernel<<<(unsigned)BN, 256, 0, st>>>(W.dPstk, S.Pstk, N, W.rf);
+        row_dot_kernel<<<(unsigned)BN, 256, 0, st>>>(W.dPstk + B * NN, S.Pstk + B * NN, N, W.rb);
+    }
     rw_bwd_kernel<<<dim3(cdiv(N, 32), cdiv(N, 32), B), 256, 0, st>>>(W.dPstk, W.dPstk + B * NN, N, S.rs, S.cs, W.rf, W.rb, dadj);
     STEP_LAUNCH_CHECK("rw_bwd");
     {
diff --git a/step_amd/csrc/optim.hip b/step_amd/csrc/optim.hip
--- a/step_amd/csrc/optim.hip
+++ b/step_amd/csrc/optim.hip
@@ -123,11 +123,18 @@
 }
 
 namespace {
+constexpr int LOSS_RING_NEXT = 6, LOSS_RING_CUR = 7, LOSS_RING_DOUBLES = 8;
 __global__ __launch_bounds__(256) void loss_reduce_kernel(const float* __restrict__ pred, const float* __restrict__ real, long n1, long rs,
                                                           float scale, float shift,
                                                           const float* __restrict__ theta, const float* __restrict__ prior, long n2,
-                                                          float null_val, double* __restrict__ acc ) {
+                                                          float null_val, double* __restrict__ acc ,
+                                                          int ring) {
     __shared__ double red[4][3];
+    if (ring) {
+        const unsigned long long call = reinterpret_cast<const unsigned long long*>(acc)[LOSS_RING_NEXT];
+        if (blockIdx.x == 0 && threadIdx.x == 0) reinterpret_cast<unsigned long long*>(acc)[LOSS_RING_CUR] = call;
+        acc += (call & 1) * 3;
+    }
     double s_abs = 0.0, s_cnt = 0.0, s_bce = 0.0;
     const long stride = (long)gridDim.x * 256;
     for (long i = (long)blockIdx.x * 256 + threadIdx.x; i < n1; i += stride) {
@@ -151,8 +158,17 @@
                                                           const float* __restrict__ theta, const float* __restrict__ prior, long n2,
                                                           float null_val, float coef, const double* __restrict__ acc,
                                                           float* __restrict__ loss, float* __restrict__ dpred, float* __restrict__ dtheta,
-                                                          const StepDynState* __restrict__ dyn) {
+                                                          const StepDynState* __restrict__ dyn, double* __restrict__ ring) {
     if (dyn) coef = dyn->gsl_coef;
+    if (ring) {
+        const unsigned long long call = reinterpret_cast<const unsigned long long*>(ring)[LOSS_RING_CUR];
+        acc = ring + (call & 1) * 3;
+        if (blockIdx.x == 0 && threadIdx.x == 0) {
+            double* other = ring + ((call + 1) & 1) * 3;
+            other[0] = 0.0; other[1] = 0.0; other[2] = 0.0;
+            reinterpret_cast<unsigned long long*>(ring)[LOSS_RING_NEXT] = call + 1;
+        }
+    }
     const double cnt = acc[1];
     const float inv_cnt = cnt > 0.0 ? (float)(1.0 / cnt) : 0.f;
     if (blockIdx.x == 0 && threadIdx.x == 0)
@@ -180,7 +196,7 @@
 
 static int loss_launch(const float* pred, const float* real, long n_pred, long real_stride, float scale, float shift, const float* theta,
                        const float* prior, long n_adj, float null_val, float coef, double* work, float* loss, float* dpred, float* dtheta,
-                       const StepDynState* dyn, void* stream);
+                       const StepDynState* dyn, void* stream, bool ring = false);
 extern "C" int step_loss_scaled_fwd_bwd(const float* pred, const float* real, long n_pred, long real_stride, float scale, float shift,
                                         const float* theta, const float* prior, long n_adj, float null_val, float coef,
                                         double* work , float* loss, float* dpred, float* dtheta, void* stream) {
@@ -192,22 +208,29 @@
     STEP_REQUIRE(dyn, "step_loss_dyn: null state");
     return loss_launch(pred, real, n_pred, real_stride, scale, shift, theta, prior, n_adj, null_val, 0.f, work, loss, dpred, dtheta, dyn, stream);
 }
+extern "C" long step_loss_ring_doubles(void) { return LOSS_RING_DOUBLES; }
+extern "C" int step_loss_ring_fwd_bwd(const float* pred, const float* real, long n_pred, long real_stride, float scale, float shift,
+                                      const float* theta, const float* prior, long n_adj, float null_val, float coef,
+                                      double* ring, float* loss, float* dpred, float* dtheta, void* stream) {
+    return loss_launch(pred, real, n_pred, real_stride, scale, shift, theta, prior, n_adj, null_val, coef, ring, loss, dpred, dtheta, nullptr, stream,
+                       step_chain_folds());
+}
 static int loss_launch(const float* pred, const float* real, long n_pred, long real_stride, float scale, float shift, const float* theta,
                        const float* prior, long n_adj, float null_val, float coef, double* work, float* loss, float* dpred, float* dtheta,
-                       const StepDynState* dyn, void* stream) {
+                       const StepDynState* dyn, void* stream, bool ring) {
     STEP_REQUIRE(pred && real && theta && prior && work && loss && dpred && dtheta && n_pred > 0 && n_adj > 0 && real_stride >= 1,
                  "step_loss: bad arguments");
     hipStream_t st = (hipStream_t)stream;
-    if (hipMemsetAsync(work, 0, 3 * sizeof(double), st) != hipSuccess) { step_set_error("step_loss: memset failed"); return STEP_ERR_HIP; }
+    if (!ring && hipMemsetAsync(work, 0, 3 * sizeof(double), st) != hipSuccess) { step_set_error("step_loss: memset failed"); return STEP_ERR_HIP; }
     long nmax = n_pred > n_adj ? n_pred : n_adj;
     int blocks = (int)((nmax + 255) / 256);
     if (blocks > 1024) blocks = 1024;
     int rblocks = (int)(nmax / 4096);
     rblocks = rblocks < 1 ? 1 : (rblocks > 1024 ? 1024 : rblocks);
-    loss_reduce_kernel<<<rblocks, 256, 0, st>>>(pred, real, n_pred, real_stride, scale, shift, theta, prior, n_adj, null_val, work);
+    loss_reduce_kernel<<<rblocks, 256, 0, st>>>(pred, real, n_pred, real_stride, scale, shift, theta, prior, n_adj, null_val, work, ring ? 1 : 0);
     STEP_LAUNCH_CHECK("loss_reduce");
     loss_finish_kernel<<<blocks, 256, 0, st>>>(pred, real, n_pred, real_stride, scale, shift, theta, prior, n_adj, null_val, coef, work, loss,
-                                               dpred, dtheta, dyn);
+                                               dpred, dtheta, dyn, ring ? work : nullptr);
     STEP_LAUNCH_CHECK("loss_finish");
     return STEP_OK;
 }
diff --git a/step_amd/csrc/step_internal.h b/step_amd/csrc/step_internal.h
--- a/step_amd/csrc/step_internal.h
+++ b/step_amd/csrc/step_internal.h
@@ -1,5 +1,6 @@
 #pragma once
 #include <hip/hip_runtime.h>
+#include <cstdlib>
 #include <vector>
 #include "../../include/step_hip.h"
 
@@ -32,6 +33,11 @@
     g.C = C; g.ldc = ldc; g.scn = 1;
     g.alpha = 1.f; g.splitk = 1;
     return g;
+}
+
+inline bool step_chain_folds() {
+    static const bool on = []() { const char* e = getenv("STEP_CHAIN_FOLDS"); return !(e && e[0] == '0'); }();
+    return on;
 }
 
 int step_gemm_rowsum_separate(StepGemm* g, hipStream_t st);
diff --git a/step_amd/step_arch/step.py b/step_amd/step_arch/step.py
--- a/step_amd/step_arch/step.py
+++ b/step_amd/step_arch/step.py
@@ -128,16 +128,18 @@
             ready.record(main)
         P = Lh // 12
         prep_done = None
-        if side is not None and model.split_wavenet_prep and model._dyn is None:
-            prep = model._side_stream(dev, "aux")
-            prep.wait_event(ready)
-            with torch.cuda.stream(prep):
-                hist.record_stream(prep)
-                L.call("step_gwnet_forward_phase_dyn", L.ptr(hist), B, N, Cin, None, None, ctypes.byref(bstruct),
-                       int(training) | (2 if (training and model.track_dead_bn7) else 0),
-                       float(drop), seed_gw, BN_MOMENTUM, L.ptr(wsaved), L.ptr(wwork), None, 5, None, L.stream())
-                prep_done = torch.cuda.Event()
-                prep_done.record(prep)
+        prefetched = side is not None and frozen is not None
+        bn_counters = [m.num_batches_tracked for m in (dgl.bn1, dgl.bn2, dgl.bn3, *list(be.bn)[:8 if model.track_dead_bn7 else 7])] if training else None
+        if prefetched and model.split_wavenet_prep and model._dyn is None:
+            if training:
+                with torch.no_grad():
+                    torch._foreach_add_(bn_counters, 1)
+                bn_counters = None
+            L.call("step_gwnet_forward_phase_dyn", L.ptr(hist), B, N, Cin, None, None, ctypes.byref(bstruct),
+                   int(training) | (2 if (training and model.track_dead_bn7) else 0),
+                   float(drop), seed_gw, BN_MOMENTUM, L.ptr(wsaved), L.ptr(wwork), None, 5, None, st)
+            prep_done = torch.cuda.Event()
+            prep_done.record(main)
 
         def graph_and_layers(sst):
             if g_kept:
@@ -162,9 +164,9 @@
             L.call("step_gwnet_forward_phase_dyn", L.ptr(hist), B, N, Cin, None, L.ptr(adj), ctypes.byref(bstruct),
                    int(training) | (2 if (training and model.track_dead_bn7) else 0),
                    float(drop), seed_gw, BN_MOMENTUM, L.ptr(wsaved), L.ptr(wwork), None, 6 if prep_done is not None else 1, L.ptr(model._dyn), sst)
-            if training:
+            if bn_counters is not None and not prefetched:
                 with torch.no_grad():
-                    torch._foreach_add_([m.num_batches_tracked for m in (dgl.bn1, dgl.bn2, dgl.bn3, *list(be.bn)[:8 if model.track_dead_bn7 else 7])], 1)
+                    torch._foreach_add_(bn_counters, 1)
 
         if frozen is None and ec is not None and ec["hit"]:
             frozen = model._eval_cache_load(ec, B, N, dev)
@@ -184,6 +186,9 @@
                 raise
         else:
             graph_and_layers(st)
+        if bn_counters is not None and prefetched:
+            with torch.no_grad():
+                torch._foreach_add_(bn_counters, 1)
         if frozen["done"] is not None:
             main.wait_event(frozen["done"])
         enc, sim, adj_knn = frozen["enc"], frozen["sim"], frozen["adj_knn"]
@@ -368,7 +373,7 @@
         self._flat_grad = None
         self._backward_count = 0
         self.overlap_streams = os.environ.get("STEP_NO_OVERLAP", "0") != "1"
-        self.split_wavenet_prep = os.environ.get("STEP_PREP_SPLIT", "0") == "1"
+        self.split_wavenet_prep = os.environ.get("STEP_PREP_SPLIT", "1") != "0"
         self.prefetch_knn_stream = os.environ.get("STEP_PREFETCH_KNN_STREAM", "0") == "1"
         self._prefetched = None
         self._precision_override = None
diff --git a/step_amd/step_loss.py b/step_amd/step_loss.py
--- a/step_amd/step_loss.py
+++ b/step_amd/step_loss.py
@@ -30,6 +30,18 @@
     return s
 
 
+_LOSS_RING = {}
+
+
+def _loss_ring(device):
+    from . import _lib
+    key = (device.index, torch.cuda.current_stream().cuda_stream)
+    w = _LOSS_RING.get(key)
+    if w is None:
+        w = _LOSS_RING[key] = torch.zeros(_lib.lib().step_loss_ring_doubles(), dtype=torch.float64, device=device)
+    return w
+
+
 class _NativeStepLoss(torch.autograd.Function):
 
     @staticmethod
@@ -44,14 +56,15 @@
         a = priori_adj.contiguous().float()
         loss = torch.empty((), device=p.device, dtype=torch.float32)
         dp, dt = torch.empty_like(p), torch.empty_like(t)
-        work = torch.empty(3, device=p.device, dtype=torch.float64)
         assert r.is_cuda and r.dtype == torch.float32
         if torch.is_tensor(coef):
+            work = torch.empty(3, device=p.device, dtype=torch.float64)
             _lib.call("step_loss_scaled_fwd_bwd_dyn", _lib.ptr(p), ctypes.c_void_p(r.data_ptr()), p.numel(), rs, float(scale), float(shift), _lib.ptr(t),
                       _lib.ptr(a), t.numel(), float(null_val), _lib.ptr(work), _lib.ptr(loss), _lib.ptr(dp), _lib.ptr(dt), _lib.ptr(coef), _lib.stream())
         else:
-            _lib.call("step_loss_scaled_fwd_bwd", _lib.ptr(p), ctypes.c_void_p(r.data_ptr()), p.numel(), rs, float(scale), float(shift), _lib.ptr(t),
-                      _lib.ptr(a), t.numel(), float(null_val), float(coef), _lib.ptr(work), _lib.ptr(loss), _lib.ptr(dp), _lib.ptr(dt), _lib.stream())
+            _lib.call("step_loss_ring_fwd_bwd", _lib.ptr(p), ctypes.c_void_p(r.data_ptr()), p.numel(), rs, float(scale), float(shift), _lib.ptr(t),
+                      _lib.ptr(a), t.numel(), float(null_val), float(coef), _lib.ptr(_loss_ring(p.device)), _lib.ptr(loss), _lib.ptr(dp), _lib.ptr(dt),
+                      _lib.stream())
         ctx.save_for_backward(dp, dt)
         ctx.shapes = (prediction.shape, theta.shape)
         return loss
```

Measured after the change: 2373, median of 6. Within noise of the previous version (+0.6%).
